# antoyang/FrozenBiLM

Hardware: AMD Instinct MI355X
Metric: video-text samples/sec (MLM fwd+bwd) DeBERTa-XL+adapters (higher is better)
Workload: dtype bf16; 1 GPU; DeBERTa-v2-XLarge(24L)+adapters ds8/8, B=32/GPU, T=10x1024, L=256 (S=266), MLM fwd+bwd+allreduce+clip+Adam, dropout 0.1 live, seeded random weights; global_batch=32, seq_len=266, parallelism=dp1, dead_layer23_encoder_pass=skipped (output unused, SURVEY fact 6); FLOPs still counted

## Files before the change

### frozenbilm_amd/attn_bwd.py

```python
from __future__ import annotations

import math

import torch

from . import lib as L

BF16, F32 = torch.bfloat16, torch.float32


_RANGE = {}


def _relidx_range(S, cfg):
    key = (S, cfg.position_buckets, cfg.max_rel, cfg.att_span)
    if key not in _RANGE:
        from .model.relpos import rel_index_vector

        rv = rel_index_vector(S, cfg.position_buckets, cfg.max_rel, cfg.att_span)
        _RANGE[key] = (int(rv[0]), int(rv[-1]) - int(rv[0]) + 1)
    return _RANGE[key]


_DRANGE = {}
POS_GRAD_MAX_DELTAS = 8


def _delta_ranges(S, cfg, dev, limit=POS_GRAD_MAX_DELTAS):
    key = (S, cfg.position_buckets, cfg.max_rel, cfg.att_span, str(dev))
    if key not in _DRANGE:
        import numpy as np

        from .model.relpos import rel_index_vector

        rv = np.asarray(rel_index_vector(S, cfg.position_buckets, cfg.max_rel, cfg.att_span), dtype=np.int64)
        rmin, rcnt = int(rv[0]), int(rv[-1]) - int(rv[0]) + 1
        first = np.searchsorted(rv, np.arange(rmin, rmin + rcnt), side="left")
        last = np.searchsorted(rv, np.arange(rmin, rmin + rcnt), side="right")
        dlo = (first - (S - 1)).astype(np.int16)
        dcnt = (last - first).astype(np.int16)
        _DRANGE[key] = (torch.from_numpy(dlo).to(dev), torch.from_numpy(dcnt).to(dev), int(dcnt.max()))
    cmax = _DRANGE[key][2]
    if limit is not None and cmax > limit:
        raise NotImplementedError(
            f"position-table gradients (fbl_attn_pos_grad) take at most {limit} relative positions per table "
            f"row; position_buckets={cfg.position_buckets}, max_relative_positions={cfg.max_rel} at sequence length {S} "
            f"puts {cmax} on one row")
    return _DRANGE[key]


def disent_attn_bwd(eng, run, sv, dctx, dqkv, dpqk, defer_pos=False):
    B, S, H, nh, span2 = run.B, run.S, eng.H, eng.nh, eng.span2
    Sp = (S + 63) // 64 * 64
    dev = eng.dev
    qkv = sv.qkv
    q, k, v = qkv[:, :H], qkv[:, H:2 * H], qkv[:, 2 * H:]
    pq, pk = sv.pqk[:, :H], sv.pqk[:, H:]
    relidx = eng.relidx(S)
    klen = getattr(run, "klen", None)
    border = getattr(run, "border", None)
    scale = 1.0 / math.sqrt(64 * 3)
    pk_ = getattr(run, "pk", None)
    row0 = pk_.row0 if pk_ is not None else None
    saved_p = getattr(sv, "psave", None) is not None

    Dv = torch.empty(B, nh, S, dtype=F32, device=dev)
    PKX = torch.empty(nh, 2 * Sp, 64, dtype=BF16, device=dev)
    if saved_p:
        QT = PQT = None
        PQX = torch.empty(nh, 2 * Sp, 64, dtype=BF16, device=dev)
    else:
        QT = torch.empty(nh, 64, B, Sp, dtype=BF16, device=dev)
        PQT = torch.empty(nh, 64, span2, dtype=BF16, device=dev)
        PQX = None
    L.attn_bwd_prep(q, pq, pk, dctx, sv.ctx, QT, PQT, Dv, B, S, Sp, nh, span2, row0=row0, relidx=relidx, PQX=PQX, PKX=PKX)
    dS = torch.empty(B, nh, Sp, Sp, dtype=BF16, device=dev)
    dST = torch.empty(B, nh, Sp, Sp, dtype=BF16, device=dev)
    lin = eng.cfg.position_buckets // 2 if eng.cfg.position_buckets > 0 else eng.cfg.att_span - 1
    if saved_p:
        L.disent_attn_bwd_dspk(sv.psave, sv.msave, q, v, dctx, PQX, sv.lse, Dv, scale, dqkv[:, H:2 * H], dqkv[:, 2 * H:], dS, dST,
                               B, S, Sp, nh, p_drop=run.p_att, seed=sv.seed_att, klen=klen, border=border, row0=row0)
        sv.psave = sv.msave = None
    else:
        lin_a = min(lin, span2 // 2) if eng.cfg.position_buckets > 0 else 0
        L.disent_attn_bwd_ds(q, k, v, dctx, pk, pq, relidx, run.mask_i32, sv.lse, Dv, scale, dqkv[:, 2 * H:], dS, dST,
                             B, S, Sp, nh, span2, p_drop=run.p_att, seed=sv.seed_att, klen=klen, border=border, lin=lin_a, row0=row0)
    L.disent_attn_bwd_dq(dS, k, PKX, dqkv[:, :H], B, S, Sp, nh, klen=klen, border=border, row0=row0)
    if not saved_p:
        L.disent_attn_bwd_shear(dST, QT, PQT, relidx, dqkv[:, H:2 * H], B, S, Sp, nh, span2, klen=klen, lin=lin, border=border,
                                row0=row0)
    rmin, rcnt = _relidx_range(S, eng.cfg)
    state = dict(dS=dS, dST=dST, q=q, k=k, rmin=rmin, rcnt=rcnt, B=B, S=S, Sp=Sp, klen=klen, row0=row0)
    if defer_pos:
        return state
    dpqk.copy_(pos_table_grads(eng, state))
    return None


def pos_table_grads(eng, st):
    H, nh, span2 = eng.H, eng.nh, eng.span2
    rmin, rcnt, B, Sp = st["rmin"], st["rcnt"], st["B"], st["Sp"]
    dpos = torch.zeros(span2, 2 * H, dtype=F32, device=eng.dev)
    dlo, dcnt, cmax = _delta_ranges(st["S"], eng.cfg, eng.dev, limit=None)
    for neg, X, Y, col0 in ((0, st["dS"], st["q"], H), (1, st["dST"], st["k"], 0)):
        d = torch.empty(1, nh, rcnt, 64, dtype=F32, device=eng.dev)
        L.attn_pos_grad(neg, [X], [Y], dlo, dcnt, cmax, d, B, st["S"], Sp, nh, rcnt, klen=st["klen"], row0=st["row0"])
        dpos[rmin:rmin + rcnt, col0:col0 + H].view(rcnt, nh, 64).copy_(d[0].permute(1, 0, 2))
    return dpos


def pos_chain_buffers(eng, run, n_exec):
    rmin, rcnt = _relidx_range(run.S, eng.cfg)
    Sp = (run.S + 63) // 64 * 64
    return dict(X1=[], X2=[], Yq=[], Yk=[], rmin=rmin, rcnt=rcnt, B=run.B, S=run.S, Sp=Sp, n=0, seeds=[], cap=n_exec, klen=None,
                row0=None)


def pos_table_grads_batched(eng, run, pc):
    H, nh, span2 = eng.H, eng.nh, eng.span2
    E, rmin, rcnt, B, Sp = pc["n"], pc["rmin"], pc["rcnt"], pc["B"], pc["Sp"]
    dev = eng.dev
    dpb = torch.empty(E, rcnt, 2 * H, dtype=BF16, device=dev)
    dlo, dcnt, cmax = _delta_ranges(pc["S"], eng.cfg, dev, limit=None)
    for neg, kx, ky, col0 in ((0, "X1", "Yq", H), (1, "X2", "Yk", 0)):
        d = torch.empty(E, nh, rcnt, 64, dtype=F32, device=dev)
        L.attn_pos_grad(neg, pc[kx][:E], pc[ky][:E], dlo, dcnt, cmax, d, B, pc["S"], Sp, nh, rcnt, klen=pc["klen"], row0=pc["row0"])
        L.heads_to_rows_bf16(d, dpb[:, :, col0:col0 + H])
    tmp = torch.empty(E, rcnt, H, dtype=F32, device=dev)
    L.gemm(dpb, eng.WposT_exec[:E], out_f32=tmp)
    dR = L.zeros(span2, H, dtype=F32, device=dev)
    L.dropout_sum_f32(tmp, pc["seeds"][:E] if run.p_hid > 0 else [0] * E, run.p_hid, dR[rmin:rmin + rcnt], key0=rmin * H)
    return dR
```

### frozenbilm_amd/csrc/attn_bwd.hip

```cpp
#include "attn_common.h"
#include "../../include/fbl.h"

namespace {
using namespace attn;

__global__ void rowdot_kernel(const bf16* dO, const bf16* O, long ld, float* out, int B, int S, int nh) {
  const long gid = (long)blockIdx.x * blockDim.x + threadIdx.x;
  const long idx = gid >> 3;
  const int c = (int)(gid & 7);
  const long total = (long)B * S * nh;
  const bool live = idx < total;
  const long row = live ? idx / nh : 0;
  const int h = live ? (int)(idx % nh) : 0;
  float s = 0.f;
  if (live) {
    const bf16x8 x = *(const bf16x8*)(dO + row * ld + h * 64 + c * 8);
    const bf16x8 y = *(const bf16x8*)(O + row * ld + h * 64 + c * 8);
#pragma unroll
    for (int e = 0; e < 8; ++e) s += bf2f(x[e]) * bf2f(y[e]);
  }
  s += __shfl_xor(s, 1, 64);
  s += __shfl_xor(s, 2, 64);
  s += __shfl_xor(s, 4, 64);
  if (live && c == 0) {
// ... 136 lines not shown
__host__ __device__ constexpr int a_total(int Sp) { return A_IDX + 2 * Sp * 2; }
static_assert(64 * LTW * 2 >= 64 * LDV * 2, "dS staging tile must fit in the T1 region");

struct ATileRegs {
  bf16x8 q[2], d[2];
  float lse, D;
};

template <bool DEVSEED, bool PACKED = false>
__global__ __launch_bounds__(256, 3) void attn_bwd_ds_kernel(BwdAArgs a) {
  extern __shared__ __attribute__((aligned(16))) char smem[];
  const int tid = threadIdx.x, lane = tid & 63;
  const int w = __builtin_amdgcn_readfirstlane(tid >> 6);
  const int c = lane & 15, g = lane >> 4;
  const int S = a.S, Sp = a.Sp;
  const WgCoord wc = wg_coord(Sp / 64, a.nh, a.B, a.border);
  const int j0 = wc.x * 64, h = wc.h, b = wc.b;
  const int j = j0 + w * 16 + c;
  const long rb = PACKED ? (long)a.row0[b] : (long)b * S;
  const int lim = PACKED ? min(a.row0[b + 1] - a.row0[b], S) : S;
  const int jc = min(j, lim - 1);
  const int tq = Sp - 1;

  int16_t* idx = (int16_t*)(smem + A_IDX);
  f16* T1 = (f16*)(smem + A_T1);
  f16* T2 = (f16*)(smem + A_T2);
  float* rlse = (float*)(smem + A_ROW);
  float* rD = rlse + 64;
  float* kms = rlse + 128;
  bf16* dst = (bf16*)(smem + A_T1);
  bf16* dstT = (bf16*)(smem + A_T2);

  const int kl = a.klen ? min(a.klen[b], S) : S;
  const int nqt = (j0 < kl) ? (kl + 63) / 64 : 0;
  const int srow = tid >> 3, sch = tid & 7;
  const int fb0 = c * 128 + ((g ^ (c & 7)) << 4), fb1 = fb0 ^ 64;
  const int sb = srow * 128 + ((sch ^ (srow & 7)) << 4);

  bf16x8 vf[2];
  {
    const long off = (rb + jc) * a.ldq + h * 64 + g * 8;
    vf[0] = *(const bf16x8*)(a.v + off);
    vf[1] = *(const bf16x8*)(a.v + off + 32);
  }
  if (nqt > 0) {
    load_idx_padded(idx, a.relidx, S, Sp, tid, 256);
#pragma unroll
    for (int t = 0; t < 2; ++t)
      *(bf16x8*)(smem + A_KS + sb + t * 4096) =
          *(const bf16x8*)(a.k + (rb + min(j0 + srow + t * 32, lim - 1)) * a.ldq + h * 64 + sch * 8);
    if (tid < 64) kms[tid] = (j0 + tid < S && a.mask[(long)b * S + min(j0 + tid, S - 1)] != 0) ? 1.f : 0.f;
    for (int t = tid; t < (2 * 64 * LTW * 2) / 16; t += 256) *(bf16x8*)(smem + A_T1 + t * 16) = (bf16x8){0, 0, 0, 0, 0, 0, 0, 0};
  }

  f32x4 dv[4];
#pragma unroll
  for (int dt = 0; dt < 4; ++dt) dv[dt] = (f32x4){0.f, 0.f, 0.f, 0.f};
  const DropKey dk = attn_drop_key(DEVSEED ? a.seed + *a.seed_dev : a.seed, b * a.nh + h, a.p_drop);
  const float k2 = a.scale * LOG2E;
  const long sbase = ((long)b * a.nh + h) * Sp * Sp;
  const int izero = a.relidx[S - 1];
  const bf16* pkh = a.pk + h * 64 + g * 8;
  const bf16* pqh = a.pq + h * 64 + g * 8;
  const int my_t0 = (0x5243 >> (w * 4)) & 15, my_t1 = (0x1670 >> (w * 4)) & 15;

  auto load_qd = [&](int it, ATileRegs& R) {
    const int i0 = it * 64;
#pragma unroll
    for (int t = 0; t < 2; ++t) {
      const int i = min(i0 + srow + t * 32, lim - 1);
      R.q[t] = *(const bf16x8*)(a.q + (rb + i) * a.ldq + h * 64 + sch * 8);
      R.d[t] = *(const bf16x8*)(a.dO + (rb + i) * a.ldo + h * 64 + sch * 8);
    }
    R.lse = INFINITY; R.D = 0.f;
    if (tid < 64) {
      const int i = i0 + tid;
      if (i < lim) {
        const long o = ((long)b * a.nh + h) * S + i;
        R.lse = a.lse[o] * LOG2E;
        R.D = a.Dv[o];
      }
    }
  };
  auto store_tile = [&](const ATileRegs& R) {
#pragma unroll
    for (int t = 0; t < 2; ++t) {
      *(bf16x8*)(smem + A_QS + sb + t * 4096) = R.q[t];
      *(bf16x8*)(smem + A_DOS + sb + t * 4096) = R.d[t];
    }
    if (tid < 64) {
      rlse[tid] = R.lse;
      rD[tid] = R.D;
    }
  };

  for (int it = 0; it < nqt; ++it) {
    const int i0 = it * 64;
    const bool band = max(abs(i0 - (j0 + 63)), abs(i0 + 63 - j0)) < a.lin;
    int r_lo, t0q[4], t0k[4];
    if (band) {
      r_lo = izero + i0 - (j0 + 63);
#pragma unroll
      for (int x = 0; x < 4; ++x) { t0q[x] = x; t0k[x] = 3 - x; }
    } else {
      if (it == 0) __syncthreads();
      r_lo = __builtin_amdgcn_readfirstlane((int)idx[i0 - (j0 + 63) + tq]);
#pragma unroll
      for (int x = 0; x < 4; ++x) {
        t0q[x] = (__builtin_amdgcn_readfirstlane((int)idx[i0 + x * 16 - (j0 + 63) + tq]) - r_lo) >> 4;
        t0k[x] = (__builtin_amdgcn_readfirstlane((int)idx[i0 - (j0 + x * 16 + 15) + tq]) - r_lo) >> 4;
      }
    }
    const int ntile = band ? 5 : 6;
    bf16x8 apk[2][2], apq[2][2];
#pragma unroll
    for (int u = 0; u < 2; ++u) {
      const long ro = (long)min(r_lo + (u ? my_t1 : my_t0) * 16 + c, a.span2 - 1) * a.ldp;
      apk[u][0] = *(const bf16x8*)(pkh + ro);
      apk[u][1] = *(const bf16x8*)(pkh + ro + 32);
      apq[u][0] = *(const bf16x8*)(pqh + ro);
      apq[u][1] = *(const bf16x8*)(pqh + ro + 32);
    }
    {
      ATileRegs R;
      load_qd(it, R);
      store_tile(R);
    }
    __syncthreads();

    f32x4 sacc[4];
    const bf16x8 kf[2] = {*(const bf16x8*)(smem + A_KS + w * 2048 + fb0), *(const bf16x8*)(smem + A_KS + w * 2048 + fb1)};
#pragma unroll
    for (int nt = 0; nt < 4; ++nt) {
      f32x4 acc = (f32x4){0.f, 0.f, 0.f, 0.f};
      acc = __builtin_amdgcn_mfma_f32_16x16x32_bf16(*(const bf16x8*)(smem + A_QS + nt * 2048 + fb0), kf[0], acc, 0, 0, 0);
      acc = __builtin_amdgcn_mfma_f32_16x16x32_bf16(*(const bf16x8*)(smem + A_QS + nt * 2048 + fb1), kf[1], acc, 0, 0, 0);
      sacc[nt] = acc;
    }
    {
      const f16 ninf = (f16)(-INFINITY);
      f16* t1s = T1 + c * LTW + g * 4;
      f16* t2s = T2 + c * LTW + g * 4;
#pragma unroll
      for (int u = 0; u < 2; ++u) {
        const int t = u ? my_t1 : my_t0;
#pragma unroll
        for (int x = 0; x < 4; ++x) {
          const int rel1 = t - t0q[x];
          if (rel1 >= 0 && rel1 < ntile) {
            f32x4 acc = (f32x4){0.f, 0.f, 0.f, 0.f};
            acc = __builtin_amdgcn_mfma_f32_16x16x32_bf16(apk[u][0], *(const bf16x8*)(smem + A_QS + x * 2048 + fb0), acc, 0, 0, 0);
            acc = __builtin_amdgcn_mfma_f32_16x16x32_bf16(apk[u][1], *(const bf16x8*)(smem + A_QS + x * 2048 + fb1), acc, 0, 0, 0);
            *(f16x4*)(t1s + x * 16 * LTW + rel1 * 16) = to_f16x4(acc);
          }
          const int rel2 = t - t0k[x];
          if (rel2 >= 0 && rel2 < ntile) {
            f32x4 acc = (f32x4){0.f, 0.f, 0.f, 0.f};
            acc = __builtin_amdgcn_mfma_f32_16x16x32_bf16(apq[u][0], *(const bf16x8*)(smem + A_KS + x * 2048 + fb0), acc, 0, 0, 0);
            acc = __builtin_amdgcn_mfma_f32_16x16x32_bf16(apq[u][1], *(const bf16x8*)(smem + A_KS + x * 2048 + fb1), acc, 0, 0, 0);
            const f16x4 tv = to_f16x4(acc);
            *(f16x4*)(t2s + x * 16 * LTW + rel2 * 16) = kms[x * 16 + c] != 0.f ? tv : (f16x4){ninf, ninf, ninf, ninf};
          }
        }
      }
    }
    __syncthreads();

    float p[16];
    if (band) {
      const f16* t1p = T1 + g * 4 * (LTW + 1) + 63 - 16 * w - c;
      const f16* t2p = T2 + (w * 16 + c) * LTW + g * 4 + 15 - c;
#pragma unroll
      for (int nt = 0; nt < 4; ++nt)
#pragma unroll
        for (int r = 0; r < 4; ++r) {
          const float s = sacc[nt][r] + (float)t1p[nt * 16 * LTW + r * (LTW + 1)] + (float)t2p[nt * 16 + r];
          p[nt * 4 + r] = __builtin_amdgcn_exp2f(fmaf(s, k2, -rlse[nt * 16 + g * 4 + r]));
        }
    } else {
      const int16_t* ib = idx + (i0 + g * 4 - j + tq);
      int sb2 = r_lo;
#pragma unroll
      for (int x = 0; x < 4; ++x) sb2 = (w == x) ? r_lo + 16 * t0k[x] : sb2;
      const f16* t1g = T1 + g * 4 * LTW;
      const f16* t2row = T2 + (w * 16 + c) * LTW;
#pragma unroll
      for (int nt = 0; nt < 4; ++nt) {
        const int sb1 = r_lo + 16 * t0q[nt];
#pragma unroll
        for (int r = 0; r < 4; ++r) {
          const int wi = ib[nt * 16 + r];
          const int w1 = clampi(wi - sb1, 0, 95), w2 = clampi(wi - sb2, 0, 95);
          const float s = sacc[nt][r] + (float)t1g[(nt * 16 + r) * LTW + w1] + (float)t2row[w2];
          p[nt * 4 + r] = __builtin_amdgcn_exp2f(fmaf(s, k2, -rlse[nt * 16 + g * 4 + r]));
        }
      }
    }
    bf16x4 dsb[4], pfh[4];
#pragma unroll
    for (int nt = 0; nt < 4; ++nt) {
      f32x4 acc = (f32x4){0.f, 0.f, 0.f, 0.f};
      acc = __builtin_amdgcn_mfma_f32_16x16x32_bf16(*(const bf16x8*)(smem + A_DOS + nt * 2048 + fb0), vf[0], acc, 0, 0, 0);
      acc = __builtin_amdgcn_mfma_f32_16x16x32_bf16(*(const bf16x8*)(smem + A_DOS + nt * 2048 + fb1), vf[1], acc, 0, 0, 0);
      float keep[4] = {1.f, 1.f, 1.f, 1.f};
      if (a.p_drop > 0.f) {
#pragma unroll
        for (int bb = 0; bb < 2; ++bb) {
          uint32_t x, y;
          attn_drop_block(dk, (i0 + nt * 16 + g * 4 + bb * 2) >> 1, j >> 1, Sp >> 1, &x, &y);
          keep[bb * 2] = attn_drop_keep(dk, x, y, 0, j & 1);
          keep[bb * 2 + 1] = attn_drop_keep(dk, x, y, 1, j & 1);
        }
      }
#pragma unroll
      for (int r = 0; r < 4; ++r) {
        const int il = nt * 16 + g * 4 + r;
        const float pv = p[nt * 4 + r];
        dsb[nt][r] = f2bf(pv * (acc[r] * keep[r] - rD[il]) * a.scale);
        pfh[nt][r] = f2bf(pv * keep[r]);
      }
    }
    __syncthreads();
#pragma unroll
    for (int kk = 0; kk < 2; ++kk) {
      bf16x8 pf;
#pragma unroll
      for (int e = 0; e < 4; ++e) {
        pf[e] = pfh[2 * kk][e];
        pf[4 + e] = pfh[2 * kk + 1][e];
      }
#pragma unroll
      for (int dt = 0; dt < 4; ++dt) {
        const int r = g * 4 + (c >> 2);
        const int ch = dt * 2 + ((c >> 1) & 1), sub = (c & 1) * 8;
        const char* db = smem + A_DOS + r * 128 + ((ch ^ (r & 7)) << 4) + sub;
        union { tr16x4 h[2]; bf16x8 v; } u;
        u.h[0] = lds_tr16((const bf16*)(db + kk * 4096));
        u.h[1] = lds_tr16((const bf16*)(db + kk * 4096 + 2048));
        dv[dt] = __builtin_amdgcn_mfma_f32_16x16x32_bf16(u.v, pf, dv[dt], 0, 0, 0);
      }
    }
#pragma unroll
    for (int nt = 0; nt < 4; ++nt) {
      *(bf16x4*)(dstT + (w * 16 + c) * LDV + nt * 16 + g * 4) = dsb[nt];
#pragma unroll
      for (int r = 0; r < 4; ++r) dst[(nt * 16 + g * 4 + r) * LDV + w * 16 + c] = dsb[nt][r];
    }
    __syncthreads();
#pragma unroll
    for (int t = 0; t < 2; ++t) {
      const int row = srow + t * 32;
      *(bf16x8*)(a.dS + sbase + (long)(i0 + row) * Sp + j0 + sch * 8) = *(const bf16x8*)(dst + row * LDV + sch * 8);
      *(bf16x8*)(a.dST + sbase + (long)(j0 + row) * Sp + i0 + sch * 8) = *(const bf16x8*)(dstT + row * LDV + sch * 8);
    }
    __syncthreads();
  }

  if (j < lim) {
    bf16* op = a.dV + (rb + j) * a.lddv + h * 64 + g * 4;
#pragma unroll
    for (int dt = 0; dt < 4; ++dt)
      *(bf16x4*)(op + dt * 16) = (bf16x4){f2bf(dv[dt][0]), f2bf(dv[dt][1]), f2bf(dv[dt][2]), f2bf(dv[dt][3])};
  }
}

struct BwdPArgs {
  const bf16* psave; const float* msave;
  const bf16* v; long ldv;
  const bf16* dO; long ldo;
  const int32_t* klen; const int32_t* border;
  const float* lse; const float* Dv;
  float scale, p_drop; uint64_t seed; const uint64_t* seed_dev;
  bf16* dV; long lddv;
  bf16* dS; bf16* dST;
  int B, S, Sp, nh;
  const int32_t* row0;
};
constexpr int LDP = 80;

__device__ __forceinline__ int tswz(int r) { return (r & 3) | ((r >> 1) & 4); }

struct BwdPKArgs {
  BwdPArgs p;
  const bf16* q; long ldq;
  const bf16* pqx;
  bf16* dK; long lddk;
};
constexpr int LDG2 = 144;
constexpr int K_DOS = 0;
constexpr int K_QS = K_DOS + 8192;
constexpr int K_PS = K_QS + 8192;
constexpr int K_STT = K_PS + 64 * LDP * 2;
constexpr int K_G2 = K_STT + 64 * LDV * 2;
constexpr int K_TAB = K_G2 + 64 * LDG2 * 2;
constexpr int K_ROW = K_TAB + 16384;
constexpr int K_TOTAL = K_ROW + 512;
static_assert(2 * K_TOTAL <= 160 * 1024, "two workgroups per CU");

struct PKTileRegs {
  bf16x8 d[2], p[2], q[2], x[2];
  float m, l, D;
};

template <bool PACKED = false>
__global__ __launch_bounds__(256, 2) void attn_bwd_dspk_kernel(BwdPKArgs ka) {
  extern __shared__ __attribute__((aligned(16))) char smem[];
  const BwdPArgs& a = ka.p;
  const int tid = threadIdx.x, lane = tid & 63;
  const int w = __builtin_amdgcn_readfirstlane(tid >> 6);
  const int c = lane & 15, g = lane >> 4;
  const int S = a.S, Sp = a.Sp;
  const WgCoord wc = wg_coord(Sp / 64, a.nh, a.B, a.border);
  const int j0 = wc.x * 64, h = wc.h, b = wc.b;
  const int j = j0 + w * 16 + c;
  const long rb = PACKED ? (long)a.row0[b] : (long)b * S;
  const int lim = PACKED ? min(a.row0[b + 1] - a.row0[b], S) : S;
  const int jc = min(j, lim - 1);
  float* rF = (float*)(smem + K_ROW);
  float* rD = rF + 64;
  bf16* dst = (bf16*)(smem + K_PS);
  bf16* dstT = (bf16*)(smem + K_STT);
  bf16* g2 = (bf16*)(smem + K_G2) + (w * 16 + c) * LDG2;

  const int kl = a.klen ? min(a.klen[b], S) : S;
  const int nqt = (j0 < kl) ? (kl + 63) / 64 : 0;
  const int srow = tid >> 3, sch = tid & 7;
  const int fb0 = c * 128 + ((g ^ (c & 7)) << 4), fb1 = fb0 ^ 64;
  const int sb = srow * 128 + ((sch ^ (srow & 7)) << 4);
  const int sp = srow * (LDP * 2) + sch * 16;
  const int sbx = srow * 128 + ((sch ^ tswz(srow)) << 4);

  bf16x8 vf[2];
  {
    const long off = (rb + jc) * a.ldv + h * 64 + g * 8;
    vf[0] = *(const bf16x8*)(a.v + off);
    vf[1] = *(const bf16x8*)(a.v + off + 32);
  }
  f32x4 dv[4], dk[4];
#pragma unroll
  for (int dt = 0; dt < 4; ++dt) {
    dv[dt] = (f32x4){0.f, 0.f, 0.f, 0.f};
    dk[dt] = (f32x4){0.f, 0.f, 0.f, 0.f};
  }
  const DropKey dkey = attn_drop_key(a.p_drop > 0.f ? fbl_seed(a.seed, a.seed_dev) : 0, b * a.nh + h, a.p_drop);
  const long sbase = ((long)b * a.nh + h) * Sp * Sp;
  const float* mrow = a.msave + (((long)b * a.nh + h) * (Sp >> 6) + wc.x) * S;
  if (nqt > 0)
    for (int t = tid; t < (64 * LDG2 * 2) / 16; t += 256) *(bf16x8*)(smem + K_G2 + t * 16) = (bf16x8){0, 0, 0, 0, 0, 0, 0, 0};
  const int W2 = 2 * Sp;
  const int ks0 = (w < 2) ? 1 : 0;
  const __amdgpu_buffer_rsrc_t xr = buf_rsrc(ka.pqx + (long)h * W2 * 64);
  const int beta0 = (Sp - j0 - 64) >> 6;
  const __amdgpu_buffer_rsrc_t dOr = buf_rsrc(a.dO + rb * a.ldo + h * 64);
  const __amdgpu_buffer_rsrc_t qr = buf_rsrc(ka.q + rb * ka.ldq + h * 64);
  const __amdgpu_buffer_rsrc_t pr = buf_rsrc(a.psave + sbase + j0);
  const __amdgpu_buffer_rsrc_t dSr = buf_rsrc(a.dS + sbase + j0);
  const __amdgpu_buffer_rsrc_t dSTr = buf_rsrc(a.dST + sbase + (long)j0 * Sp);
  const uint32_t ldo2 = (uint32_t)(a.ldo * 2), ldq2 = (uint32_t)(ka.ldq * 2);
  const uint32_t po = (uint32_t)((srow * Sp + sch * 8) * 2);
  auto load_tile = [&](int it, PKTileRegs& R) {
    const int i0 = it * 64;
#pragma unroll
    for (int t = 0; t < 2; ++t) {
      const uint32_t ir = (uint32_t)min(i0 + srow + t * 32, lim - 1);
      R.d[t] = buf_ld16(dOr, ir * ldo2 + (uint32_t)(sch * 16), 0);
      R.p[t] = buf_ld16(pr, po + (uint32_t)(t * 32 * Sp * 2), (uint32_t)(i0 * Sp * 2));
    }
#pragma unroll
    for (int t = 0; t < 2; ++t) R.x[t] = buf_ld16(xr, (uint32_t)((srow + t * 32) * 128 + sch * 16), (uint32_t)((beta0 + it + 1) * 8192));
    {
      const int i = min(i0 + lane, lim - 1);
      const long o = ((long)b * a.nh + h) * S + i;
      R.l = a.lse[o];
      R.m = mrow[i];
      R.D = a.Dv[o];
    }
  };
  auto load_q = [&](int it, PKTileRegs& R) {
#pragma unroll
    for (int t = 0; t < 2; ++t) {
      const uint32_t ir = (uint32_t)min(it * 64 + srow + t * 32, lim - 1);
      R.q[t] = (FBL_ATTN_DBGBITS & 16) ? vf[0] : buf_ld16(qr, ir * ldq2 + (uint32_t)(sch * 16), 0);
    }
  };
  auto store_tile = [&](const PKTileRegs& R, int it_i0) {
#pragma unroll
    for (int t = 0; t < 2; ++t) {
      *(bf16x8*)(smem + K_DOS + sb + t * 4096) = R.d[t];
      *(bf16x8*)(smem + K_QS + sb + t * 4096) = R.q[t];
      *(bf16x8*)(smem + K_TAB + (((it_i0 >> 6) + beta0 + 1) & 1) * 8192 + sbx + t * 4096) = R.x[t];
      *(bf16x8*)(smem + K_PS + sp + t * (32 * LDP * 2)) = R.p[t];
    }
    if (tid < 64) {
      const bool live = it_i0 + tid < lim && R.l < INFINITY;
      rF[tid] = live ? __builtin_amdgcn_exp2f(R.m - R.l * LOG2E) : 0.f;
      rD[tid] = live ? R.D : 0.f;
    }
  };

  PKTileRegs R;
  if (nqt > 0) {
    load_tile(0, R);
    load_q(0, R);
#pragma unroll
    for (int t = 0; t < 2; ++t)
      *(bf16x8*)(smem + K_TAB + (beta0 & 1) * 8192 + sbx + t * 4096) =
          buf_ld16(xr, (uint32_t)((srow + t * 32) * 128 + sch * 16), (uint32_t)(beta0 * 8192));
  }
  for (int it = 0; it < nqt; ++it) {
    const int i0 = it * 64;
    store_tile(R, i0);
    __syncthreads();
    {
      const int itn = min(it + 1, nqt - 1);
      load_tile(itn, R);
      load_q(itn, R);
    }

    bf16x4 dsb[4], pfh[4];
#pragma unroll
    for (int nt = 0; nt < 4; ++nt) {
      union { tr16x4 t; bf16x4 v; } pu;
      pu.t = lds_tr16((const bf16*)(smem + K_PS + (nt * 16 + g * 4 + (c >> 2)) * (LDP * 2) + (w * 16 + (c & 3) * 4) * 2));
      const f32x4 f4 = *(const f32x4*)(rF + nt * 16 + g * 4);
      const f32x4 d4 = *(const f32x4*)(rD + nt * 16 + g * 4);
      f32x4 acc = (f32x4){0.f, 0.f, 0.f, 0.f};
      acc = __builtin_amdgcn_mfma_f32_16x16x32_bf16(*(const bf16x8*)(smem + K_DOS + nt * 2048 + fb0), vf[0], acc, 0, 0, 0);
      acc = __builtin_amdgcn_mfma_f32_16x16x32_bf16(*(const bf16x8*)(smem + K_DOS + nt * 2048 + fb1), vf[1], acc, 0, 0, 0);
      float keep[4];
#pragma unroll
      for (int r = 0; r < 4; ++r) keep[r] = pu.t[r] < 0 ? 0.f : dkey.inv_keep;
#pragma unroll
      for (int r = 0; r < 4; ++r) {
        const float pv = f4[r] != 0.f ? fabsf(bf2f(pu.v[r])) * f4[r] : 0.f;
        dsb[nt][r] = f2bf(pv * (acc[r] * keep[r] - d4[r]) * a.scale);
        pfh[nt][r] = f2bf(pv * keep[r]);
      }
    }
#pragma unroll
    for (int kk = 0; kk < 2; ++kk) {
      bf16x8 pf, sf;
#pragma unroll
      for (int e = 0; e < 4; ++e) {
        pf[e] = pfh[2 * kk][e];
        pf[4 + e] = pfh[2 * kk + 1][e];
        sf[e] = dsb[2 * kk][e];
        sf[4 + e] = dsb[2 * kk + 1][e];
      }
#pragma unroll
      for (int dt = 0; dt < 4; ++dt) {
        const int r = g * 4 + (c >> 2);
        const int ch = dt * 2 + ((c >> 1) & 1), sub = (c & 1) * 8;
        const int o = r * 128 + ((ch ^ (r & 7)) << 4) + sub + kk * 4096;
        union { tr16x4 h[2]; bf16x8 v; } u, uq;
        u.h[0] = lds_tr16((const bf16*)(smem + K_DOS + o));
        u.h[1] = lds_tr16((const bf16*)(smem + K_DOS + o + 2048));
        dv[dt] = __builtin_amdgcn_mfma_f32_16x16x32_bf16(u.v, pf, dv[dt], 0, 0, 0);
        if (FBL_ATTN_DBGBITS & 2) continue;
        uq.h[0] = lds_tr16((const bf16*)(smem + K_QS + o));
        uq.h[1] = lds_tr16((const bf16*)(smem + K_QS + o + 2048));
        dk[dt] = __builtin_amdgcn_mfma_f32_16x16x32_bf16(uq.v, sf, dk[dt], 0, 0, 0);
      }
    }
    {
      bf16* gs = g2 + 64 - (w * 16 + c) + g * 4;
#pragma unroll
      for (int nt = 0; nt < 4; ++nt) {
        *(bf16x4*)(dstT + (w * 16 + c) * LDV + nt * 16 + g * 4) = dsb[nt];
#pragma unroll
        for (int r = 0; r < 4; ++r) {
          dst[(nt * 16 + g * 4 + r) * LDP + w * 16 + c] = dsb[nt][r];
          if (!(FBL_ATTN_DBGBITS & 4)) gs[nt * 16 + r] = dsb[nt][r];
        }
      }
    }
    if (!(FBL_ATTN_DBGBITS & 8)) {
#pragma unroll
      for (int u = 0; u < 3; ++u) {
        const int x0 = (ks0 + u) * 32 + g * 8;
        const int slot = (((i0 >> 6) + beta0 + (x0 >> 6)) & 1) * 8192;
        const int r = (x0 & 63) + (c >> 2);
        const bf16x8 gf = *(const bf16x8*)(g2 + (ks0 + u) * 32 + g * 8);
#pragma unroll
        for (int dt = 0; dt < 4; ++dt) {
          const int ch = dt * 2 + ((c >> 1) & 1), sub = (c & 1) * 8;
          union { tr16x4 h[2]; bf16x8 v; } ut;
          ut.h[0] = lds_tr16((const bf16*)(smem + K_TAB + slot + r * 128 + ((ch ^ tswz(r)) << 4) + sub));
          ut.h[1] = lds_tr16((const bf16*)(smem + K_TAB + slot + (r + 4) * 128 + ((ch ^ tswz(r + 4)) << 4) + sub));
          dk[dt] = __builtin_amdgcn_mfma_f32_16x16x32_bf16(ut.v, gf, dk[dt], 0, 0, 0);
        }
      }
    }
    __syncthreads();
#pragma unroll
    for (int t = 0; t < 2; ++t) {
      const int row = srow + t * 32;
      buf_st16(dSr, po + (uint32_t)(t * 32 * Sp * 2), (uint32_t)(i0 * Sp * 2), *(const bf16x8*)(dst + row * LDP + sch * 8));
      buf_st16(dSTr, po + (uint32_t)(t * 32 * Sp * 2), (uint32_t)(i0 * 2), *(const bf16x8*)(dstT + row * LDV + sch * 8));
    }
  }

  if (j < lim) {
    bf16* op = a.dV + (rb + j) * a.lddv + h * 64 + g * 4;
    bf16* ok = ka.dK + (rb + j) * ka.lddk + h * 64 + g * 4;
#pragma unroll
    for (int dt = 0; dt < 4; ++dt) {
      *(bf16x4*)(op + dt * 16) = (bf16x4){f2bf(dv[dt][0]), f2bf(dv[dt][1]), f2bf(dv[dt][2]), f2bf(dv[dt][3])};
      *(bf16x4*)(ok + dt * 16) = (bf16x4){f2bf(dk[dt][0]), f2bf(dk[dt][1]), f2bf(dk[dt][2]), f2bf(dk[dt][3])};
    }
  }
}

struct BwdQArgs {
  const bf16* dS;
  const bf16* k; long ldk;
  const bf16* pkx;
  const int32_t* klen; const int32_t* border;
  bf16* dQ; long lddq;
  int B, S, Sp, nh;
  const int32_t* row0;
};
constexpr int LDG1 = 104;
constexpr int Q_DS = 0;
constexpr int Q_KS = Q_DS + 8192;
constexpr int Q_G1 = Q_KS + 8192;
constexpr int Q_TAB = Q_G1 + 64 * LDG1 * 2;
constexpr int Q_TOTAL = Q_TAB + 16384;
static_assert(3 * Q_TOTAL <= 160 * 1024, "three workgroups per CU");

template <bool PACKED = false>
__global__ __launch_bounds__(256, 3) void attn_bwd_dq_kernel(BwdQArgs a) {
  extern __shared__ __attribute__((aligned(16))) char smem[];
  const int tid = threadIdx.x, lane = tid & 63;
  const int w = __builtin_amdgcn_readfirstlane(tid >> 6);
  const int c = lane & 15, g = lane >> 4;
  const int S = a.S, Sp = a.Sp;
  const WgCoord wc = wg_coord(Sp / 64, a.nh, a.B, a.border);
  const int i0 = wc.x * 64, h = wc.h, b = wc.b;
  const int i = i0 + w * 16 + c;
  const long rb = PACKED ? (long)a.row0[b] : (long)b * S;
  const int lim = PACKED ? min(a.row0[b + 1] - a.row0[b], S) : S;
  const int kl = a.klen ? min(a.klen[b], S) : S;
  const int nkt = (i0 < kl) ? (kl + 63) / 64 : 0;
  const int srow = tid >> 3, sch = tid & 7;
  const int sb = srow * 128 + ((sch ^ tswz(srow)) << 4);
  const int ks0 = (w < 2) ? 0 : 1;
  bf16* g1 = (bf16*)(smem + Q_G1) + (w * 16 + c) * LDG1;
  const int wr = w * 16 + c;
  f32x4 dq[4];
#pragma unroll
  for (int dt = 0; dt < 4; ++dt) dq[dt] = (f32x4){0.f, 0.f, 0.f, 0.f};
  if (nkt > 0) {
    for (int t = tid; t < (64 * LDG1 * 2) / 16; t += 256) *(bf16x8*)(smem + Q_G1 + t * 16) = (bf16x8){0, 0, 0, 0, 0, 0, 0, 0};
    __syncthreads();
  }

  const long sbase = ((long)b * a.nh + h) * Sp * Sp;
  const __amdgpu_buffer_rsrc_t sr = buf_rsrc(a.dS + sbase + (long)i0 * Sp);
  const __amdgpu_buffer_rsrc_t kr = buf_rsrc(a.k + rb * a.ldk + h * 64);
  const __amdgpu_buffer_rsrc_t xr = buf_rsrc(a.pkx + (long)h * 2 * Sp * 64);
  const uint32_t so = (uint32_t)((wr * Sp + g * 16) * 2);
  const uint32_t ldk2 = (uint32_t)(a.ldk * 2);
  const int beta0 = (i0 - 64 + Sp) >> 6;

  struct Regs { bf16x8 s[2], k[2], x[2]; } R;
  auto load_pair = [&](int jt) {
#pragma unroll
    for (int t = 0; t < 2; ++t) {
      R.s[t] = buf_ld16(sr, so + (uint32_t)(t * 16), (uint32_t)(jt * 128));
      const uint32_t jr = (uint32_t)min(jt * 64 + srow + t * 32, lim - 1);
      R.k[t] = buf_ld16(kr, jr * ldk2 + (uint32_t)(sch * 16), 0);
      R.x[t] = buf_ld16(xr, (uint32_t)((srow + t * 32) * 128 + sch * 16), (uint32_t)((beta0 - jt) * 8192));
    }
  };
  if (nkt > 0) {
    load_pair(0);
#pragma unroll
    for (int t = 0; t < 2; ++t)
      *(bf16x8*)(smem + Q_TAB + ((beta0 + 1) & 1) * 8192 + sb + t * 4096) =
          buf_ld16(xr, (uint32_t)((srow + t * 32) * 128 + sch * 16), (uint32_t)((beta0 + 1) * 8192));
  }
  for (int jt = 0; jt < nkt; ++jt) {
#pragma unroll
    for (int t = 0; t < 2; ++t) {
      *(bf16x8*)(smem + Q_KS + sb + t * 4096) = R.k[t];
      *(bf16x8*)(smem + Q_TAB + ((beta0 - jt) & 1) * 8192 + sb + t * 4096) = R.x[t];
      *(bf16x8*)(smem + Q_DS + wr * 128 + (((2 * g + t) ^ (wr & 7)) << 4)) = R.s[t];
    }
    {
      bf16* gs = g1 + wr + 64 - g * 16 - ks0 * 32;
#pragma unroll
      for (int t = 0; t < 2; ++t)
#pragma unroll
        for (int e = 0; e < 8; ++e) gs[-(t * 8 + e)] = R.s[t][e];
    }
    __syncthreads();
    load_pair(min(jt + 1, nkt - 1));
#pragma unroll
    for (int kk = 0; kk < 2; ++kk) {
      const int rk = kk * 32 + g * 8 + (c >> 2);
      const bf16x8 sf = *(const bf16x8*)(smem + Q_DS + wr * 128 + (((kk * 4 + g) ^ (wr & 7)) << 4));
#pragma unroll
      for (int dt = 0; dt < 4; ++dt) {
        const int ch = dt * 2 + ((c >> 1) & 1), sub = (c & 1) * 8;
        union { tr16x4 h[2]; bf16x8 v; } u;
        u.h[0] = lds_tr16((const bf16*)(smem + Q_KS + rk * 128 + ((ch ^ tswz(rk)) << 4) + sub));
        u.h[1] = lds_tr16((const bf16*)(smem + Q_KS + (rk + 4) * 128 + ((ch ^ tswz(rk + 4)) << 4) + sub));
        dq[dt] = __builtin_amdgcn_mfma_f32_16x16x32_bf16(u.v, sf, dq[dt], 0, 0, 0);
      }
    }
#pragma unroll
    for (int u3 = 0; u3 < 3; ++u3) {
      const int x0 = (ks0 + u3) * 32 + g * 8;
      const int slot = ((beta0 - jt + (x0 >> 6)) & 1) * 8192;
      const int r = (x0 & 63) + (c >> 2);
      const bf16x8 gf = *(const bf16x8*)(g1 + u3 * 32 + g * 8);
#pragma unroll
      for (int dt = 0; dt < 4; ++dt) {
        const int ch = dt * 2 + ((c >> 1) & 1), sub = (c & 1) * 8;
        union { tr16x4 h[2]; bf16x8 v; } ut;
        ut.h[0] = lds_tr16((const bf16*)(smem + Q_TAB + slot + r * 128 + ((ch ^ tswz(r)) << 4) + sub));
        ut.h[1] = lds_tr16((const bf16*)(smem + Q_TAB + slot + (r + 4) * 128 + ((ch ^ tswz(r + 4)) << 4) + sub));
        dq[dt] = __builtin_amdgcn_mfma_f32_16x16x32_bf16(ut.v, gf, dq[dt], 0, 0, 0);
      }
    }
    __syncthreads();
  }
  if (i < lim) {
    bf16* op = a.dQ + (rb + i) * a.lddq + h * 64 + g * 4;
#pragma unroll
    for (int dt = 0; dt < 4; ++dt)
      *(bf16x4*)(op + dt * 16) = (bf16x4){f2bf(dq[dt][0]), f2bf(dq[dt][1]), f2bf(dq[dt][2]), f2bf(dq[dt][3])};
  }
}

struct ShearArgs {
  const bf16* X;
  const bf16* YT; long y_sh, y_sb, y_sd;
  const bf16* PT;
  const int16_t* relidx;
  const int32_t* klen;
  const int32_t* border;
  bf16* out; long ldout;
  int B, S, Sp, nh, span2, Wg;
  int lin;
  const int32_t* row0;
};
__device__ __forceinline__ void gt_window(const int16_t* relidx, int S, int kl, int r0, int Wg, int* rbase, int* nks) {
  const int hi = 2 * S - 2;
  const int dlo = -(r0 + 31), dhi = kl - 1 - r0;
  const int rb = (int)relidx[min(max(dlo + S - 1, 0), hi)] & ~7;
  const int rt = (int)relidx[min(max(dhi + S - 1, 0), hi)];
  *rbase = rb;
  *nks = min((rt - rb + 32) / 32, Wg / 32);
}
constexpr int C_IDX = 0;
constexpr int C_G = C_IDX + 2048;

template <bool PACKED = false>
__global__ __launch_bounds__(128) void attn_bwd_shear_kernel(ShearArgs a) {
  extern __shared__ __attribute__((aligned(16))) char smem[];
  const int tid = threadIdx.x, lane = tid & 63;
  const int w = __builtin_amdgcn_readfirstlane(tid >> 6);
  const int c = lane & 15, g = lane >> 4;
  const int S = a.S, Sp = a.Sp;
  const WgCoord wc = wg_coord(Sp / 32, a.nh, a.B, a.border);
  const int r0 = wc.x * 32, h = wc.h, b = wc.b;
  const int LDG = a.Wg + 8;
  const int rl = w * 16 + c;
  const int row = r0 + rl;
  bf16* G = (bf16*)(smem + C_G);
  int16_t* idx = (int16_t*)(smem + C_IDX);
  const bf16x8 z8 = {0, 0, 0, 0, 0, 0, 0, 0};
  const int kl = a.klen ? min(a.klen[b], S) : S;
  const long rb = PACKED ? (long)a.row0[b] : (long)b * S;
  const int lim = PACKED ? min(a.row0[b + 1] - a.row0[b], S) : S;
  if (r0 >= kl) {
    if (row < lim) {
      bf16* op = a.out + (rb + row) * a.ldout + h * 64 + g * 4;
#pragma unroll
      for (int dt = 0; dt < 4; ++dt) *(bf16x4*)(op + dt * 16) = (bf16x4){0, 0, 0, 0};
    }
    return;
  }
  int rbase, nks;
  gt_window(a.relidx, S, kl, r0, a.Wg, &rbase, &nks);
  const int izero = (int)a.relidx[S - 1];
  {
    const int vpr = nks * 4;
    for (int t = tid; t < 32 * vpr; t += 128) *(bf16x8*)(G + (t / vpr) * LDG + (t % vpr) * 8) = z8;
  }
  attn::load_idx_padded(idx, a.relidx, S, Sp, tid, 128);
  const long xbase = (((long)b * a.nh + h) * Sp + row) * Sp;
  f32x4 acc[4];
#pragma unroll
  for (int dt = 0; dt < 4; ++dt) acc[dt] = (f32x4){0.f, 0.f, 0.f, 0.f};
  __syncthreads();

  const int nct = (kl + 63) / 64;
  const bf16* ytb = a.YT + h * a.y_sh + b * a.y_sb + (long)c * a.y_sd + g * 8;
  const int16_t* ib = idx + (Sp - 1 - row + g * 8);
  bf16* grow = G + rl * LDG - rbase;
  const int wmax = rbase + nks * 32 - 1;
  const int dummy = rbase + a.Wg;
  const int lin0 = izero + g * 8 - row;
  const int rw = r0 + w * 16;
  struct Frags { bf16x8 y[8], x[2]; };
  auto load_ct = [&](int ct, Frags& F) {
    const int c0 = ct * 64;
#pragma unroll
    for (int kk = 0; kk < 2; ++kk)
#pragma unroll
      for (int dt = 0; dt < 4; ++dt)
        F.y[kk * 4 + dt] = (FBL_ATTN_DBGBITS & 2048) ? z8 : *(const bf16x8*)(ytb + (long)(dt * 16) * a.y_sd + c0 + kk * 32);
    F.x[0] = *(const bf16x8*)(a.X + xbase + c0 + g * 8);
    F.x[1] = *(const bf16x8*)(a.X + xbase + c0 + 32 + g * 8);
  };
  auto step = [&](int ct, const Frags& F) {
    const int c0 = ct * 64;
    const int d_a = rw - (c0 + 63), d_b = rw + 15 - c0;
    const bool band = max(abs(d_a), abs(d_b)) < a.lin;
#pragma unroll
    for (int kk = 0; kk < 2; ++kk) {
      const bf16x8 xv = F.x[kk];
#pragma unroll
      for (int dt = 0; dt < 4; ++dt) acc[dt] = __builtin_amdgcn_mfma_f32_16x16x32_bf16(F.y[kk * 4 + dt], xv, acc[dt], 0, 0, 0);
      const int cb = c0 + kk * 32;
      if (FBL_ATTN_DBGBITS & 512) continue;
      if (band) {
        const int s0 = lin0 + cb;
#pragma unroll
        for (int e = 0; e < 8; ++e) {
          const int slot = s0 + e;
          grow[bf2f(xv[e]) != 0.f ? slot : dummy] = xv[e];
        }
      } else {
#pragma unroll
        for (int e = 0; e < 8; ++e) {
          const float x = bf2f(xv[e]);
          if (x != 0.f) {
            const int dlt = cb + g * 8 + e - row;
            const int gi = clampi((int)ib[cb + e], rbase, wmax);
            if (abs(dlt) < a.lin) {
              grow[gi] = xv[e];
            } else {
              bf16x2 pv = {(bf16)0.f, (bf16)0.f};
              pv[gi & 1] = xv[e];
              __builtin_amdgcn_ds_atomic_fadd_v2bf16((__attribute__((address_space(3))) bf16x2*)(grow + (gi & ~1)), pv);
            }
          }
        }
      }
    }
  };
  {
    Frags F0, F1;
    load_ct(0, F0);
    for (int ct = 0; ct < nct; ct += 2) {
      if (ct + 1 < nct) load_ct(ct + 1, F1);
      step(ct, F0);
      if (ct + 2 < nct) load_ct(ct + 2, F0);
      if (ct + 1 < nct) step(ct + 1, F1);
    }
  }
  const bf16* pt = a.PT + (long)h * 64 * a.span2 + rbase + g * 8;
  auto load_pt = [&](int kk, bf16x8* dstf) {
#pragma unroll
    for (int dt = 0; dt < 4; ++dt) {
      const bool ok = rbase + kk * 32 + g * 8 + 8 <= a.span2;
      dstf[dt] = ok ? *(const bf16x8*)(pt + (long)(dt * 16 + c) * a.span2 + kk * 32) : z8;
    }
  };
  auto table_step = [&](int kk, const bf16x8* af) {
    const bf16x8 bfv = *(const bf16x8*)(G + rl * LDG + kk * 32 + g * 8);
#pragma unroll
    for (int dt = 0; dt < 4; ++dt) acc[dt] = __builtin_amdgcn_mfma_f32_16x16x32_bf16(af[dt], bfv, acc[dt], 0, 0, 0);
  };
  bf16x8 pa[4], pb[4];
  const int nks_run = (FBL_ATTN_DBGBITS & 1024) ? 0 : nks;
  load_pt(0, pa);
  for (int kk = 0; kk < nks_run; kk += 2) {
    if (kk + 1 < nks) load_pt(kk + 1, pb);
    table_step(kk, pa);
    if (kk + 2 < nks) load_pt(kk + 2, pa);
    if (kk + 1 < nks) table_step(kk + 1, pb);
  }
  if (row < lim) {
    bf16* op = a.out + (rb + row) * a.ldout + h * 64 + g * 4;
#pragma unroll
    for (int dt = 0; dt < 4; ++dt)
      *(bf16x4*)(op + dt * 16) = (bf16x4){f2bf(acc[dt][0]), f2bf(acc[dt][1]), f2bf(acc[dt][2]), f2bf(acc[dt][3])};
  }
}

constexpr int PG_MAX_E = 64;
struct PosGradArgs {
  const bf16* X[PG_MAX_E];
  const bf16* Y[PG_MAX_E];
  long ldy;
  const int16_t* dlo;
  const int16_t* dcnt;
  const int32_t* klen;
  const int32_t* row0;
  float* out;
  int E, B, S, Sp, nh, rcnt;
  int cmax;
};
constexpr int PG_PAD = 48;
constexpr int PG_LDY = 80;
constexpr int PG_TPW = 4;
constexpr int PG_WAVES = 4, PG_THR = PG_WAVES * 64;
constexpr int PG_ROWS = PG_WAVES * PG_TPW * 16;
__host__ __device__ constexpr int pg_pitch(int Sp) { return Sp + 2 * PG_PAD; }
__host__ __device__ constexpr int pg_buf(int Sp) { return 32 * pg_pitch(Sp) * 2 + 32 * PG_LDY * 2; }
__host__ __device__ constexpr int pg_smem(int Sp) { return 2 * pg_buf(Sp); }

template <bool NEG, int CM, int NXR, int OCC>
__global__ __launch_bounds__(PG_THR, OCC) void pos_grad_kernel(PosGradArgs a) {
  extern __shared__ __attribute__((aligned(16))) char smem[];
  const int tid = threadIdx.x, lane = tid & 63;
  const int w = __builtin_amdgcn_readfirstlane(tid >> 6);
  const int c = lane & 15, g = lane >> 4;
  const int S = a.S, Sp = a.Sp, P = pg_pitch(Sp);
  const int nsplit = (a.rcnt + PG_ROWS - 1) / PG_ROWS;
  const int L8 = blockIdx.x >> 3, xcd = blockIdx.x & 7;
  const int prob = (L8 / nsplit) * 8 + xcd, part = L8 % nsplit;
  if (prob >= a.E * a.nh) return;
  const int e = prob / a.nh, h = prob % a.nh;
  const int bufsz = pg_buf(Sp);
  const bf16* X = a.X[e];
  const bf16* Y = a.Y[e];
  const int ntiles = (a.rcnt + 15) / 16;

  int d0[PG_TPW], dn[PG_TPW], tlo[PG_TPW], thi[PG_TPW];
  bool simple[PG_TPW];
#pragma unroll
  for (int u = 0; u < PG_TPW; ++u) {
    const int t = (w + PG_WAVES * u) * nsplit + part;
    const int r = min(t * 16 + c, a.rcnt - 1);
    const bool live = t < ntiles && t * 16 + c < a.rcnt;
    d0[u] = live ? (int)a.dlo[r] : 0;
    dn[u] = live ? (int)a.dcnt[r] : 0;
    const int rf = min(t * 16, a.rcnt - 1), rl = min(t * 16 + 15, a.rcnt - 1);
    tlo[u] = t < ntiles ? (int)a.dlo[rf] : 1 << 20;
    thi[u] = t < ntiles ? (int)a.dlo[rl] + (int)a.dcnt[rl] - 1 : -(1 << 20);
    simple[u] = t < ntiles && t * 16 + 15 < a.rcnt && (thi[u] - tlo[u]) == 15 && __builtin_amdgcn_ballot_w64(dn[u] != 1) == 0;
  }
  f32x4 acc[PG_TPW][4];
#pragma unroll
  for (int u = 0; u < PG_TPW; ++u)
#pragma unroll
    for (int dt = 0; dt < 4; ++dt) acc[u][dt] = (f32x4){0.f, 0.f, 0.f, 0.f};

  for (int id = tid; id < (OCC >= 3 ? 1 : 2) * 32 * 2 * (PG_PAD / 8); id += PG_THR) {
    const int bsel = id / (32 * 2 * (PG_PAD / 8)), r2 = id % (32 * 2 * (PG_PAD / 8));
    const int row = r2 / (2 * (PG_PAD / 8)), q = r2 % (2 * (PG_PAD / 8));
    const int col = q < PG_PAD / 8 ? q * 8 : PG_PAD + Sp + (q - PG_PAD / 8) * 8;
    *(bf16x8*)((bf16*)(smem + bsel * bufsz) + row * P + col) = (bf16x8){0, 0, 0, 0, 0, 0, 0, 0};
  }
  const bf16x8 z8 = (bf16x8){0, 0, 0, 0, 0, 0, 0, 0};
  const int srow = tid >> 3, sch = tid & 7, nq = Sp >> 6;

  int b_n = 0, k_n = 0, kl_n = 0;
  auto seek = [&]() {
    while (b_n < a.B) {
      kl_n = a.klen ? min(a.klen[b_n], S) : S;
      if (k_n < kl_n) return true;
      ++b_n; k_n = 0;
    }
    return false;
  };
  bf16x8 rx[NXR], ry;
  int it_b = 0, it_k = 0, it_kl = 0;
  auto load_item = [&]() {
    it_b = b_n; it_k = k_n; it_kl = kl_n;
    const int kl64 = (kl_n + 63) & ~63;
    const long rb = a.row0 ? (long)a.row0[b_n] : (long)b_n * S;
    const int lim = a.row0 ? min(a.row0[b_n + 1] - a.row0[b_n], S) : S;
    const bf16* Xb = X + (((long)b_n * a.nh + h) * Sp) * Sp + (long)k_n * Sp;
    const bf16* xr = Xb + (long)srow * Sp + sch * 8;
#pragma unroll
    for (int q = 0; q < NXR; ++q) rx[q] = (q < nq && sch * 8 + q * 64 < kl64) ? *(const bf16x8*)(xr + q * 64) : z8;
    {
      const int pos = k_n + srow;
      ry = (pos < lim) ? *(const bf16x8*)(Y + (rb + pos) * a.ldy + h * 64 + sch * 8) : z8;
    }
    k_n += 32;
  };
  int pb = 0;
  bool have = seek();
  if (have) load_item();
  while (have) {
    bf16* xs = (bf16*)(smem + pb * bufsz);
    bf16* ys = xs + 32 * P;
    if (OCC >= 3) __syncthreads();
    {
      bf16* xw = xs + srow * P + PG_PAD + sch * 8;
#pragma unroll
      for (int q = 0; q < NXR; ++q)
        if (q < nq) *(bf16x8*)(xw + q * 64) = rx[q];
    }
    *(bf16x8*)(ys + srow * PG_LDY + sch * 8) = ry;
    const int k0 = it_k, kl = it_kl;
    __syncthreads();
    have = seek();
    if (have) load_item();
    bf16x8 yf[4];
#pragma unroll
    for (int dt = 0; dt < 4; ++dt) {
      const bf16* yb = ys + (g * 8 + (c >> 2)) * PG_LDY + dt * 16 + (c & 3) * 4;
      union { tr16x4 hh[2]; bf16x8 v; } u2;
      u2.hh[0] = lds_tr16(yb);
      u2.hh[1] = lds_tr16(yb + 4 * PG_LDY);
      yf[dt] = u2.v;
    }
#pragma unroll
    for (int u = 0; u < PG_TPW; ++u) {
      const int cmin = NEG ? k0 + tlo[u] : k0 - thi[u];
      const int cmax = NEG ? k0 + 31 + thi[u] : k0 + 31 - tlo[u];
      if (cmax < 0 || cmin >= kl) continue;
      bf16x8 gf;
      const bf16* xrow = xs + (g * 8) * P + PG_PAD;
      const int cb = NEG ? (k0 + g * 8 + d0[u]) : (k0 + g * 8 - d0[u]);
      if (simple[u]) {
#pragma unroll
        for (int q = 0; q < 8; ++q) gf[q] = xrow[q * P + cb + q];
      } else {
        const int lo = -PG_PAD, hi = Sp + PG_PAD - 1;
        bf16 vv[8][CM];
#pragma unroll
        for (int q = 0; q < 8; ++q)
#pragma unroll
          for (int t2 = 0; t2 < CM; ++t2) vv[q][t2] = xrow[q * P + clampi(NEG ? cb + q + t2 : cb + q - t2, lo, hi)];
#pragma unroll
        for (int q = 0; q < 8; ++q) {
          float sum = 0.f;
#pragma unroll
          for (int t2 = 0; t2 < CM; ++t2) sum += t2 < dn[u] ? bf2f(vv[q][t2]) : 0.f;
          gf[q] = f2bf(sum);
        }
      }
#pragma unroll
      for (int dt = 0; dt < 4; ++dt) acc[u][dt] = __builtin_amdgcn_mfma_f32_16x16x32_bf16(yf[dt], gf, acc[u][dt], 0, 0, 0);
    }
    if (OCC < 3) pb ^= 1;
  }
  float* ob = a.out + ((long)e * a.nh + h) * a.rcnt * 64;
#pragma unroll
  for (int u = 0; u < PG_TPW; ++u) {
    const int r = ((w + PG_WAVES * u) * nsplit + part) * 16 + c;
    if (r < a.rcnt) {
#pragma unroll
      for (int dt = 0; dt < 4; ++dt) *(f32x4*)(ob + (long)r * 64 + dt * 16 + g * 4) = acc[u][dt];
    }
  }
}

constexpr int PGW_PAD = 6;
__host__ __device__ constexpr int pgw_pitch(int Sp) { return Sp + PGW_PAD; }
__host__ __device__ constexpr int pgw_smem(int Sp) { return 32 * pgw_pitch(Sp) * 4 + 32 * PG_LDY * 2; }

template <bool NEG>
__global__ __launch_bounds__(PG_THR, 2) void pos_grad_wide_kernel(PosGradArgs a) {
  extern __shared__ __attribute__((aligned(16))) char smem[];
  const int tid = threadIdx.x, lane = tid & 63;
  const int w = __builtin_amdgcn_readfirstlane(tid >> 6);
  const int c = lane & 15, g = lane >> 4;
  const int S = a.S, Sp = a.Sp, PP = pgw_pitch(Sp);
  const int nsplit = (a.rcnt + PG_ROWS - 1) / PG_ROWS;
  const int L8 = blockIdx.x >> 3, xcd = blockIdx.x & 7;
  const int prob = (L8 / nsplit) * 8 + xcd, part = L8 % nsplit;
  if (prob >= a.E * a.nh) return;
  const int e = prob / a.nh, h = prob % a.nh;
  float* cs = (float*)smem;
  bf16* ys = (bf16*)(smem + 32 * PP * 4);
  const bf16* X = a.X[e];
  const bf16* Y = a.Y[e];
  const int ntiles = (a.rcnt + 15) / 16;

  int d0[PG_TPW], dn[PG_TPW], tlo[PG_TPW], thi[PG_TPW];
#pragma unroll
  for (int u = 0; u < PG_TPW; ++u) {
    const int t = (w + PG_WAVES * u) * nsplit + part;
    const int r = min(t * 16 + c, a.rcnt - 1);
    const bool live = t < ntiles && t * 16 + c < a.rcnt;
    d0[u] = live ? (int)a.dlo[r] : 0;
    dn[u] = live ? (int)a.dcnt[r] : 0;
    const int rf = min(t * 16, a.rcnt - 1), rl = min(t * 16 + 15, a.rcnt - 1);
    tlo[u] = t < ntiles ? (int)a.dlo[rf] : 1 << 20;
    thi[u] = t < ntiles ? (int)a.dlo[rl] + (int)a.dcnt[rl] - 1 : -(1 << 20);
  }
  f32x4 acc[PG_TPW][4];
#pragma unroll
  for (int u = 0; u < PG_TPW; ++u)
#pragma unroll
    for (int dt = 0; dt < 4; ++dt) acc[u][dt] = (f32x4){0.f, 0.f, 0.f, 0.f};

  if (tid < 32) cs[tid * PP + 1] = 0.f;
  const bf16x8 z8 = (bf16x8){0, 0, 0, 0, 0, 0, 0, 0};
  const int srow = tid >> 3, sch = tid & 7, nq = Sp >> 6;

  int b_n = 0, k_n = 0, kl_n = 0;
  auto seek = [&]() {
    while (b_n < a.B) {
      kl_n = a.klen ? min(a.klen[b_n], S) : S;
      if (k_n < kl_n) return true;
      ++b_n; k_n = 0;
    }
    return false;
  };
  bf16x8 rx[8], ry;
  int it_k = 0, it_kl = 0;
  auto load_item = [&]() {
    it_k = k_n; it_kl = kl_n;
    const int kl64 = (kl_n + 63) & ~63;
    const long rb = a.row0 ? (long)a.row0[b_n] : (long)b_n * S;
    const int lim = a.row0 ? min(a.row0[b_n + 1] - a.row0[b_n], S) : S;
    const bf16* xr = X + (((long)b_n * a.nh + h) * Sp) * Sp + (long)(k_n + srow) * Sp + sch * 8;
#pragma unroll
    for (int q = 0; q < 8; ++q) rx[q] = (q < nq && sch * 8 + q * 64 < kl64) ? *(const bf16x8*)(xr + q * 64) : z8;
    const int pos = k_n + srow;
    ry = (pos < lim) ? *(const bf16x8*)(Y + (rb + pos) * a.ldy + h * 64 + sch * 8) : z8;
    k_n += 32;
  };
  bool have = seek();
  if (have) load_item();
  while (have) {
    __syncthreads();
    {
      float* cw = cs + srow * PP + 2 + sch * 8;
      float carry = 0.f;
#pragma unroll
      for (int q = 0; q < 8; ++q) {
        if (q < nq) {
          float run[8];
          run[0] = bf2f(rx[q][0]);
#pragma unroll
          for (int i = 1; i < 8; ++i) run[i] = run[i - 1] + bf2f(rx[q][i]);
          float incl = run[7];
#pragma unroll
          for (int s = 1; s < 8; s <<= 1) {
            const float o = __shfl_up(incl, s, 8);
            if (sch >= s) incl += o;
          }
          const float excl = __shfl_up(incl, 1, 8);
          const float base = carry + (sch ? excl : 0.f);
#pragma unroll
          for (int i = 0; i < 8; i += 2) *(float2*)(cw + q * 64 + i) = make_float2(base + run[i], base + run[i + 1]);
          carry += __shfl(incl, 7, 8);
        }
      }
    }
    *(bf16x8*)(ys + srow * PG_LDY + sch * 8) = ry;
    const int k0 = it_k, kl = it_kl;
    __syncthreads();
    have = seek();
    if (have) load_item();
    bf16x8 yf[4];
#pragma unroll
    for (int dt = 0; dt < 4; ++dt) {
      const bf16* yb = ys + (g * 8 + (c >> 2)) * PG_LDY + dt * 16 + (c & 3) * 4;
      union { tr16x4 hh[2]; bf16x8 v; } u2;
      u2.hh[0] = lds_tr16(yb);
      u2.hh[1] = lds_tr16(yb + 4 * PG_LDY);
      yf[dt] = u2.v;
    }
    const float* crow = cs + (g * 8) * PP + 1;
#pragma unroll
    for (int u = 0; u < PG_TPW; ++u) {
      const int cmin = NEG ? k0 + tlo[u] : k0 - thi[u];
      const int cmax = NEG ? k0 + 31 + thi[u] : k0 + 31 - tlo[u];
      if (cmax < 0 || cmin >= kl) continue;
      const int kb = k0 + g * 8;
      float hi[8], lo[8];
#pragma unroll
      for (int q = 0; q < 8; ++q) {
        const int jl = NEG ? kb + q + d0[u] : kb + q - d0[u] - dn[u] + 1;
        hi[q] = crow[q * PP + clampi(jl + dn[u], 0, Sp)];
        lo[q] = crow[q * PP + clampi(jl, 0, Sp)];
      }
      bf16x8 gf;
#pragma unroll
      for (int q = 0; q < 8; ++q) gf[q] = f2bf(hi[q] - lo[q]);
#pragma unroll
      for (int dt = 0; dt < 4; ++dt) acc[u][dt] = __builtin_amdgcn_mfma_f32_16x16x32_bf16(yf[dt], gf, acc[u][dt], 0, 0, 0);
    }
  }
  float* ob = a.out + ((long)e * a.nh + h) * a.rcnt * 64;
#pragma unroll
  for (int u = 0; u < PG_TPW; ++u) {
    const int r = ((w + PG_WAVES * u) * nsplit + part) * 16 + c;
    if (r < a.rcnt) {
#pragma unroll
      for (int dt = 0; dt < 4; ++dt) *(f32x4*)(ob + (long)r * 64 + dt * 16 + g * 4) = acc[u][dt];
    }
  }
}

}

extern "C" int fbl_attn_rowdot(const void* dO, const void* O, int64_t ld, float* out, int B, int S, int nh,
                               void* stream) {
  if (ld % 8) return FBL_ERR_ALIGN;
  const long total = (long)B * S * nh;
  if (total <= 0) return 0;
  hipLaunchKernelGGL(rowdot_kernel, dim3((unsigned)((total * 8 + 255) / 256)), dim3(256), 0, (hipStream_t)stream,
                     (const bf16*)dO, (const bf16*)O, (long)ld, out, B, S, nh);
  FBL_CHECK_LAUNCH();
  return 0;
}

extern "C" int fbl_disent_attn_bwd_ds(const void* q, const void* k, const void* v, int64_t ldq, const void* dO,
                                      int64_t ldo,
                                      const void* pk, const void* pq, int64_t ldp, const int16_t* relidx,
                                      const int32_t* mask, const int32_t* klen, const int32_t* border, const float* lse, const float* Dv, float scale, float p_drop,
                                      uint64_t seed, const uint64_t* seed_dev, void* dV, int64_t lddv, void* dS, void* dST, int B, int S, int Sp,
                                      int nh, int span2, int lin_span, const int32_t* row0, void* stream) {
  if (S < 1 || S > 512 || Sp < S || Sp % 64) return FBL_ERR_SHAPE;
  if ((ldq % 8) || (ldo % 8) || (ldp % 8) || (lddv % 4)) return FBL_ERR_ALIGN;
  if (lin_span < 0 || 2 * lin_span > span2) return FBL_ERR_ARG;
  if (row0 && !klen) return FBL_ERR_ARG;
  if (B <= 0 || nh <= 0) return 0;
  BwdAArgs a{(const bf16*)q, (const bf16*)k, (const bf16*)v, ldq, (const bf16*)dO, ldo, (const bf16*)pk, (const bf16*)pq, ldp, relidx, mask, klen, border, lse, Dv, scale, p_drop, seed, (bf16*)dV, lddv,
             (bf16*)dS, (bf16*)dST, B, S, Sp, nh, span2, lin_span, seed_dev, row0};
  attn_debug_init();
  const int smem_bytes = a_total(Sp);
  static int attr_bytes = 0;
  if (smem_bytes > attr_bytes) {
    hipError_t e = hipFuncSetAttribute((const void*)attn_bwd_ds_kernel<false>, hipFuncAttributeMaxDynamicSharedMemorySize, smem_bytes);
    if (e == hipSuccess) e = hipFuncSetAttribute((const void*)attn_bwd_ds_kernel<true>, hipFuncAttributeMaxDynamicSharedMemorySize, smem_bytes);
    if (e == hipSuccess) e = hipFuncSetAttribute((const void*)attn_bwd_ds_kernel<false, true>, hipFuncAttributeMaxDynamicSharedMemorySize, smem_bytes);
    if (e == hipSuccess) e = hipFuncSetAttribute((const void*)attn_bwd_ds_kernel<true, true>, hipFuncAttributeMaxDynamicSharedMemorySize, smem_bytes);
    if (e != hipSuccess) return (int)e;
    attr_bytes = smem_bytes;
  }
  const dim3 grid((unsigned)(Sp / 64) * nh * B);
  const bool devseed = seed_dev && p_drop > 0.f;
  if (row0 && devseed)
    hipLaunchKernelGGL((attn_bwd_ds_kernel<true, true>), grid, dim3(256), smem_bytes, (hipStream_t)stream, a);
  else if (row0)
    hipLaunchKernelGGL((attn_bwd_ds_kernel<false, true>), grid, dim3(256), smem_bytes, (hipStream_t)stream, a);
  else if (devseed)
    hipLaunchKernelGGL(attn_bwd_ds_kernel<true>, grid, dim3(256), smem_bytes, (hipStream_t)stream, a);
  else
    hipLaunchKernelGGL(attn_bwd_ds_kernel<false>, grid, dim3(256), smem_bytes, (hipStream_t)stream, a);
  FBL_CHECK_LAUNCH();
  return 0;
}

extern "C" int fbl_disent_attn_bwd_dspk(const void* psave, const float* msave, const void* q, int64_t ldq, const void* v, int64_t ldv,
                                        const void* dO, int64_t ldo, const void* pqx, const int32_t* klen, const int32_t* border,
                                        const float* lse, const float* Dv, float scale, float p_drop, uint64_t seed,
                                        const uint64_t* seed_dev, void* dK, int64_t lddk, void* dV, int64_t lddv, void* dS, void* dST,
                                        int B, int S, int Sp, int nh, const int32_t* row0, void* stream) {
  if (S < 1 || S > 512 || Sp < S || Sp % 64) return FBL_ERR_SHAPE;
  if ((ldv % 8) || (ldo % 8) || (ldq % 8) || (lddv % 4) || (lddk % 4)) return FBL_ERR_ALIGN;
  if (!psave || !msave || !q || !v || !dO || !pqx || !lse || !Dv || !dK || !dV || !dS || !dST) return FBL_ERR_ARG;
  if (row0 && !klen) return FBL_ERR_ARG;
  if (B <= 0 || nh <= 0) return 0;
  BwdPKArgs a{{(const bf16*)psave, msave, (const bf16*)v, ldv, (const bf16*)dO, ldo, klen, border, lse, Dv, scale, p_drop, seed,
               seed_dev, (bf16*)dV, lddv, (bf16*)dS, (bf16*)dST, B, S, Sp, nh, row0},
              (const bf16*)q, ldq, (const bf16*)pqx, (bf16*)dK, lddk};
  attn_debug_init();
  static bool attr_set = false;
  if (!attr_set) {
    hipError_t e = hipFuncSetAttribute((const void*)attn_bwd_dspk_kernel<false>, hipFuncAttributeMaxDynamicSharedMemorySize, K_TOTAL);
    if (e == hipSuccess) e = hipFuncSetAttribute((const void*)attn_bwd_dspk_kernel<true>, hipFuncAttributeMaxDynamicSharedMemorySize, K_TOTAL);
    if (e != hipSuccess) return (int)e;
    attr_set = true;
  }
  const dim3 grid((unsigned)(Sp / 64) * nh * B);
  if (row0)
    hipLaunchKernelGGL(attn_bwd_dspk_kernel<true>, grid, dim3(256), K_TOTAL, (hipStream_t)stream, a);
  else
    hipLaunchKernelGGL(attn_bwd_dspk_kernel<false>, grid, dim3(256), K_TOTAL, (hipStream_t)stream, a);
  FBL_CHECK_LAUNCH();
  return 0;
}

extern "C" int fbl_disent_attn_bwd_dq(const void* dS, const void* k, int64_t ldk, const void* pkx, const int32_t* klen,
                                      const int32_t* border, void* dQ, int64_t lddq, int B, int S, int Sp, int nh,
                                      const int32_t* row0, void* stream) {
  if (S < 1 || S > 512 || Sp < S || Sp % 64) return FBL_ERR_SHAPE;
  if ((ldk % 8) || (lddq % 4)) return FBL_ERR_ALIGN;
  if (!dS || !k || !pkx || !dQ) return FBL_ERR_ARG;
  if (row0 && !klen) return FBL_ERR_ARG;
  if (B <= 0 || nh <= 0) return 0;
  BwdQArgs a{(const bf16*)dS, (const bf16*)k, ldk, (const bf16*)pkx, klen, border, (bf16*)dQ, lddq, B, S, Sp, nh, row0};
  static bool attr_set = false;
  if (!attr_set) {
    hipError_t e = hipFuncSetAttribute((const void*)attn_bwd_dq_kernel<false>, hipFuncAttributeMaxDynamicSharedMemorySize, Q_TOTAL);
    if (e == hipSuccess) e = hipFuncSetAttribute((const void*)attn_bwd_dq_kernel<true>, hipFuncAttributeMaxDynamicSharedMemorySize, Q_TOTAL);
    if (e != hipSuccess) return (int)e;
    attr_set = true;
  }
  const dim3 grid((unsigned)(Sp / 64) * nh * B);
  if (row0)
    hipLaunchKernelGGL(attn_bwd_dq_kernel<true>, grid, dim3(256), Q_TOTAL, (hipStream_t)stream, a);
  else
    hipLaunchKernelGGL(attn_bwd_dq_kernel<false>, grid, dim3(256), Q_TOTAL, (hipStream_t)stream, a);
  FBL_CHECK_LAUNCH();
  return 0;
}

extern "C" int fbl_disent_attn_bwd_shear(const void* dST, const void* QT, int64_t y_sh, int64_t y_sb, int64_t y_sd,
                                         const void* PQT, const int16_t* relidx, const int32_t* klen, const int32_t* border,
                                         void* dK, int64_t lddk, int lin_span, int B, int S, int Sp, int nh, int span2,
                                         const int32_t* row0, void* stream) {
  if (S < 1 || S > 512 || Sp < S || Sp % 64 || span2 > 512 || span2 % 32) return FBL_ERR_SHAPE;
  if ((lddk % 4) || (y_sd % 8) || (y_sb % 8) || (y_sh % 8)) return FBL_ERR_ALIGN;
  if (B <= 0 || nh <= 0) return 0;
  int Wg = S + 31 + 7;
  if (Wg > span2) Wg = span2;
  Wg = (Wg + 31) / 32 * 32;
  if (row0 && !klen) return FBL_ERR_ARG;
  ShearArgs a{(const bf16*)dST, (const bf16*)QT, y_sh, y_sb, y_sd, (const bf16*)PQT, relidx, klen, border, (bf16*)dK, lddk,
              B, S, Sp, nh, span2, Wg, lin_span, row0};
  attn_debug_init();
  const int smem_bytes = C_G + 32 * (Wg + 8) * 2;
  static int attr_bytes = 0;
  if (smem_bytes > attr_bytes) {
    hipError_t e = hipFuncSetAttribute((const void*)attn_bwd_shear_kernel<false>, hipFuncAttributeMaxDynamicSharedMemorySize, smem_bytes);
    if (e == hipSuccess) e = hipFuncSetAttribute((const void*)attn_bwd_shear_kernel<true>, hipFuncAttributeMaxDynamicSharedMemorySize, smem_bytes);
    if (e != hipSuccess) return (int)e;
    attr_bytes = smem_bytes;
  }
  dim3 grid((unsigned)(Sp / 32) * nh * B);
  if (row0)
    hipLaunchKernelGGL(attn_bwd_shear_kernel<true>, grid, dim3(128), smem_bytes, (hipStream_t)stream, a);
  else
    hipLaunchKernelGGL(attn_bwd_shear_kernel<false>, grid, dim3(128), smem_bytes, (hipStream_t)stream, a);
  FBL_CHECK_LAUNCH();
  return 0;
}

extern "C" int fbl_attn_pos_grad(int neg, const void* const* X, const void* const* Y, int64_t ldy, const int16_t* dlo,
                                 const int16_t* dcnt, int dcnt_max, const int32_t* klen, const int32_t* row0, float* out, int E,
                                 int B, int S, int Sp, int nh, int rcnt, void* stream) {
  if (S < 1 || S > 512 || Sp < S || Sp % 64 || rcnt < 1 || rcnt > 1024) return FBL_ERR_SHAPE;
  if (ldy % 8) return FBL_ERR_ALIGN;
  if (!X || !Y || !dlo || !dcnt || !out || dcnt_max < 1) return FBL_ERR_ARG;
  if (row0 && !klen) return FBL_ERR_ARG;
  if (E <= 0 || B <= 0 || nh <= 0) return 0;
  for (int e = 0; e < E; ++e)
    if (!X[e] || !Y[e]) return FBL_ERR_ARG;
  static const int occ_sw = FBL_ENV_INT("FBL_POSGRAD_OCC", 3);
  const bool occ3 = Sp <= 320 && dcnt_max <= 3 && occ_sw >= 3;
  const int smem_bytes = occ3 ? pg_buf(Sp) : pg_smem(Sp);
  static int attr_bytes = 0;
  if (pg_smem(Sp) > attr_bytes) {
    const void* fns[6] = {(const void*)pos_grad_kernel<false, 3, 5, 3>, (const void*)pos_grad_kernel<true, 3, 5, 3>,
                          (const void*)pos_grad_kernel<false, 3, 8, 2>, (const void*)pos_grad_kernel<true, 3, 8, 2>,
                          (const void*)pos_grad_kernel<false, 8, 8, 2>, (const void*)pos_grad_kernel<true, 8, 8, 2>};
    for (int i = 0; i < 6; ++i) {
      hipError_t e1 = hipFuncSetAttribute(fns[i], hipFuncAttributeMaxDynamicSharedMemorySize, pg_smem(Sp));
      if (e1 != hipSuccess) return (int)e1;
    }
    attr_bytes = pg_smem(Sp);
  }
  const bool wide = dcnt_max > 8;
  static int attr_wide = 0;
  if (wide && pgw_smem(Sp) > attr_wide) {
    for (const void* fn : {(const void*)pos_grad_wide_kernel<false>, (const void*)pos_grad_wide_kernel<true>}) {
      hipError_t e1 = hipFuncSetAttribute(fn, hipFuncAttributeMaxDynamicSharedMemorySize, pgw_smem(Sp));
      if (e1 != hipSuccess) return (int)e1;
    }
    attr_wide = pgw_smem(Sp);
  }
  const int nsplit = (rcnt + PG_ROWS - 1) / PG_ROWS;
  for (int e0 = 0; e0 < E; e0 += PG_MAX_E) {
    PosGradArgs a{};
    const int ne = E - e0 < PG_MAX_E ? E - e0 : PG_MAX_E;
    for (int e = 0; e < ne; ++e) {
      a.X[e] = (const bf16*)X[e0 + e];
      a.Y[e] = (const bf16*)Y[e0 + e];
    }
    a.ldy = ldy; a.dlo = dlo; a.dcnt = dcnt; a.klen = klen; a.row0 = row0;
    a.out = out + (long)e0 * nh * rcnt * 64;
    a.E = ne; a.B = B; a.S = S; a.Sp = Sp; a.nh = nh; a.rcnt = rcnt; a.cmax = dcnt_max;
    const dim3 grid((unsigned)(((ne * nh + 7) / 8) * 8 * nsplit));
#define FBL_PG_LAUNCH(NEG_, CM_, NXR_, OCC_) \
  hipLaunchKernelGGL((pos_grad_kernel<NEG_, CM_, NXR_, OCC_>), grid, dim3(PG_THR), smem_bytes, (hipStream_t)stream, a)
    if (wide) {
      if (neg) hipLaunchKernelGGL(pos_grad_wide_kernel<true>, grid, dim3(PG_THR), pgw_smem(Sp), (hipStream_t)stream, a);
      else hipLaunchKernelGGL(pos_grad_wide_kernel<false>, grid, dim3(PG_THR), pgw_smem(Sp), (hipStream_t)stream, a);
    } else if (occ3) {
      if (neg) FBL_PG_LAUNCH(true, 3, 5, 3);
      else FBL_PG_LAUNCH(false, 3, 5, 3);
    } else if (dcnt_max <= 3) {
      if (neg) FBL_PG_LAUNCH(true, 3, 8, 2);
      else FBL_PG_LAUNCH(false, 3, 8, 2);
    } else {
      if (neg) FBL_PG_LAUNCH(true, 8, 8, 2);
      else FBL_PG_LAUNCH(false, 8, 8, 2);
    }
#undef FBL_PG_LAUNCH
    FBL_CHECK_LAUNCH();
  }
  return 0;
}

extern "C" int fbl_attn_bwd_prep(const void* q, int64_t ldq, const void* pq, const void* pk, int64_t ldp, const void* dO,
                                 const void* O, int64_t ldo, void* QT, void* PQT, float* Dv, const int16_t* relidx, void* PQX,
                                 void* PKX, int B, int S, int Sp, int nh, int span2, const int32_t* row0, void* stream) {
  if (S < 1 || Sp < S || Sp % 64 || span2 <= 0 || span2 % 64) return FBL_ERR_SHAPE;
  if ((ldq % 8) || (ldp % 8) || (ldo % 8)) return FBL_ERR_ALIGN;
  if ((PQX || PKX) && !relidx) return FBL_ERR_ARG;
  if (!Dv) return FBL_ERR_ARG;
  if (B <= 0 || nh <= 0) return 0;
  const int n_tr = (Sp / 64) * nh * B, n_tab = (span2 / 64) * nh, n_x = (2 * Sp / 64) * nh;
  PrepArgs a{(const bf16*)q, ldq, (const bf16*)pq, (const bf16*)pk, ldp, (const bf16*)dO, (const bf16*)O, ldo, (bf16*)QT,
             (bf16*)PQT, Dv, B, S, Sp, nh, span2, QT ? n_tr : 0, PQT ? n_tab : 0, row0, relidx, (bf16*)PQX, (bf16*)PKX,
             PQX ? n_x : 0, PKX ? n_x : 0};
  const long n_dot = ((long)B * S * nh * 8 + 255) / 256;
  const long grid = (long)a.n_qt + a.n_pqt + a.n_pqx + a.n_pkx + n_dot;
  hipLaunchKernelGGL(attn_bwd_prep_kernel, dim3((unsigned)grid), dim3(256), 0, (hipStream_t)stream, a);
  FBL_CHECK_LAUNCH();
  return 0;
}
```

### frozenbilm_amd/engine.py

```python
from __future__ import annotations

import math
from dataclasses import dataclass, field
from typing import Dict, List, Optional

import numpy as np
import torch

from . import lib as L
from .model.relpos import rel_index_vector

BF16, F32 = torch.bfloat16, torch.float32


def _ru(x: int, m: int) -> int:
    return (x + m - 1) // m * m


@dataclass
class NormRef:
    t: torch.Tensor
    stats: torch.Tensor
    gamma: torch.Tensor
    beta: torch.Tensor
    rowmask: Optional[torch.Tensor] = None

    def as_args(self):
        return (self.t, self.stats, self.gamma, self.beta, self.rowmask)


@dataclass
class Stream:
    bf16: torch.Tensor
    norm: Optional[NormRef] = None
    plain: Optional[torch.Tensor] = None
    full: Optional[torch.Tensor] = None


@dataclass
class Packing:
    row0: torch.Tensor
    sel: torch.Tensor
    inv: torch.Tensor
    pos: torch.Tensor
    n: int


class Engine:
    def __init__(self, model):
        self.m = model
        cfg = model.config
        self.cfg = cfg
        self.H, self.I, self.V = cfg.hidden_size, cfg.intermediate_size, cfg.vocab_size
        self.nh = cfg.num_attention_heads
        self.nL = cfg.num_hidden_layers
        self.span2 = 2 * cfg.att_span
        self.lin_span = min(cfg.position_buckets // 2, cfg.att_span) if cfg.position_buckets > 0 else 0
        self.F = model.features_dim
        self.Fp = _ru(self.F, 64) if self.F else 0
        self.A1 = self.H // model.ds_factor_attn if model.ds_factor_attn else 0
        self.A2 = self.H // model.ds_factor_ff if model.ds_factor_ff else 0
        self.Vp = _ru(self.V, 64)
        dev = model.device
        if dev.type != "cuda":
            raise RuntimeError("frozenbilm_amd runs on MI355X only: move the model to a cuda (HIP) device; "
                               "there is no CPU fallback")
        L.load()
        self.dev = dev
        self.opts = dict(getattr(model, "engine_options", None) or {})
        unknown = set(self.opts) - {"eager_logits", "side_stream", "fold_dx", "dw_on_side", "fuse_tail", "merge", "dw_group", "attn_save_p"}
        if unknown:
            raise ValueError(f"unknown engine_options: {sorted(unknown)}")
        self._build_flat()
        self._pack_frozen()
        self._relidx: Dict[int, torch.Tensor] = {}
        self._pos_cache: Dict[int, torch.Tensor] = {}
        self._no_pos_cache = False
        self.reducer = None
        self._pad_bufs = {}
        self._dyz_pool: Dict[tuple, list] = {}
        self._dyz_shape = None
        self.params_version = 0
        self._ops_version = None
        self.skip_dead_layer = True
        self._ln_ws = L.ln_bwd_ws(self.H, dev)
        self._cs_ws = L.colsum_ws(max(self.H, self.I), dev)
        self.sk_ws = torch.empty(48 << 20, dtype=F32, device=dev)
        self.side = torch.cuda.Stream(device=dev)
        if L._AUX.get(dev.index if dev.index is not None else torch.cuda.current_device()) is None:
            L.set_aux_stream(torch.cuda.Stream(device=dev), dev)
        o = self.opts
        self.eager_logits = bool(o.get("eager_logits", False))
        self.side_ws = torch.empty(8 << 20, dtype=F32, device=dev)
        self.side_cs_ws = L.colsum_ws(max(self.H, self.I), dev)
        self.use_side_stream = bool(o.get("side_stream", True))
        self.fold_dx = bool(o.get("fold_dx", True))
        self.dw_on_side = bool(o.get("dw_on_side", False))
        self.attn_save_p = bool(o.get("attn_save_p", True))
        self.fuse_tail = bool(o.get("fuse_tail", True))
        L.exclude_from_aux(self.side)
        self.dw_group = max(1, min(L.ADW_MAX_ADAPTERS, int(o.get("dw_group", 16))))

    def _build_flat(self):
        from .model.deberta import flat_order

        m = self.m
        named = dict(m.named_parameters())
        train_names = [n for n, p in named.items() if p.requires_grad]
        order = flat_order(self.cfg, train_names)
        offs, total = {}, 0
        for n in order:
            offs[n] = total
            total += _ru(named[n].numel(), 8)
        self.flat = torch.zeros(total, dtype=F32, device=self.dev)
        from .parallel import SCALAR_SLOT

        self.flat_grad_full = torch.zeros(SCALAR_SLOT + total, dtype=F32, device=self.dev)
        self.flat_grad = self.flat_grad_full[SCALAR_SLOT:]
        self.flat_bf16 = torch.zeros(total, dtype=BF16, device=self.dev)
        self.offsets, self.order = offs, order
        self._adT_offs = {}
        self.G: Dict[str, torch.Tensor] = {}
        self.Pb: Dict[str, torch.Tensor] = {}
        for n in order:
            p = named[n]
            o, k = offs[n], p.numel()
            view = self.flat[o:o + k].view(p.shape)
            view.copy_(p.data)
            p.data = view
            self.G[n] = self.flat_grad[o:o + k].view(p.shape)
            self.Pb[n] = self.flat_bf16[o:o + k].view(p.shape)
        self.P = {n: p.data for n, p in named.items()}
        self.named = named
        self.bucket_ends: Dict[str, int] = {}
        for n in order:
            key = self._bucket_key(n)
            self.bucket_ends[key] = offs[n] + _ru(named[n].numel(), 8)

    def _bucket_key(self, name: str) -> str:
        if name.startswith("lm_predictions."):
            return "head"
        if name.startswith("deberta.encoder.layer."):
            return "layer" + name.split(".")[3]
        if name.startswith("deberta.encoder.conv."):
            return "layer0" if False else "conv"
        if name.startswith("deberta.encoder.LayerNorm"):
            return "relln"
        return "emb"

    def attach_grads(self):
        fresh = all(self.named[n].grad is None for n in self.order)
        if fresh:
            L.zero_(self.flat_grad)
        for n in self.order:
            p = self.named[n]
            if p.grad is None:
                if not fresh:
                    self.G[n].zero_()
                p.grad = self.G[n]
            elif p.grad.data_ptr() != self.G[n].data_ptr():
                self.G[n].copy_(p.grad)
                p.grad = self.G[n]

    def _pack_frozen(self):
        P, H, I = self.P, self.H, self.I
        nL, dev = self.nL, self.dev
        bf = lambda t: t.to(BF16).contiguous()
        self.merge1 = bool(self.A1) and self.A1 % 64 == 0 and H % 64 == 0 and bool(self.opts.get("merge", True))
        self.merge2 = bool(self.A2) and self.A2 % 64 == 0 and H % 64 == 0 and bool(self.opts.get("merge", True))
        self.WoT_rev = torch.empty(nL, H, H, dtype=BF16, device=dev)
        self.WdT_rev = torch.empty(nL, I, H, dtype=BF16, device=dev)
        if self.merge1:
            self.Kf1 = _ru(H + self.A1, 128)
            self.WoF_rev = torch.zeros(nL, H, self.Kf1, dtype=BF16, device=dev)
            self.WoM_rev = torch.zeros(nL, H + self.A1, H, dtype=BF16, device=dev)
            self.boM_rev = torch.zeros(nL, H + self.A1, dtype=F32, device=dev)
            self.bo16_rev = torch.zeros(nL, 1, H, dtype=BF16, device=dev)
        if self.merge2:
            self.WdM_rev = torch.zeros(nL, H + self.A2, I, dtype=BF16, device=dev)
            self.bdM_rev = torch.zeros(nL, H + self.A2, dtype=F32, device=dev)
            self.bd16_rev = torch.zeros(nL, 1, H, dtype=BF16, device=dev)
        self.Lw = []
        for i in range(self.nL):
            p = f"deberta.encoder.layer.{i}"
            s = p + ".attention.self."
            j = nL - 1 - i
            Wqkv = torch.cat([P[s + "query_proj.weight"], P[s + "key_proj.weight"], P[s + "value_proj.weight"]], 0)
            self.WoT_rev[j].copy_(P[p + ".attention.output.dense.weight"].t())
            self.WdT_rev[j].copy_(P[p + ".output.dense.weight"].t())
            d = dict(
                Wqkv=bf(Wqkv), WqkvT=bf(Wqkv.t()),
                bqkv=torch.cat([P[s + "query_proj.bias"], P[s + "key_proj.bias"], P[s + "value_proj.bias"]]).float().contiguous(),
                Wo=bf(P[p + ".attention.output.dense.weight"]), WoT=self.WoT_rev[j],
                bo=P[p + ".attention.output.dense.bias"].float().contiguous(),
                Wi=bf(P[p + ".intermediate.dense.weight"]), WiT=bf(P[p + ".intermediate.dense.weight"].t()),
                bi=P[p + ".intermediate.dense.bias"].float().contiguous(),
                Wd=bf(P[p + ".output.dense.weight"]), WdT=self.WdT_rev[j],
                bd=P[p + ".output.dense.bias"].float().contiguous(),
            )
            if self.merge1:
                self.WoM_rev[j, :H].copy_(d["Wo"])
                self.boM_rev[j, :H].copy_(d["bo"])
                self.bo16_rev[j, 0].copy_(d["bo"])
                d["WoM"], d["boM"] = self.WoM_rev[j], self.boM_rev[j]
                self.WoF_rev[j, :, :H].copy_(self.WoT_rev[j])
                d["WoF"] = self.WoF_rev[j]
            if self.merge2:
                self.WdM_rev[j, :H].copy_(d["Wd"])
                self.bdM_rev[j, :H].copy_(d["bd"])
                self.bd16_rev[j, 0].copy_(d["bd"])
                d["WdM"], d["bdM"] = self.WdM_rev[j], self.bdM_rev[j]
            self.Lw.append(d)
        order = [nL - 1, nL - 1] + list(range(nL - 2, -1, -1))
        self.WposT_exec = torch.empty(len(order), H, 2 * H, dtype=BF16, device=dev)
        for e, li in enumerate(order):
            self.WposT_exec[e].copy_(self.Lw[li]["WqkvT"][:, : 2 * H])
        if self.cfg.conv_kernel_size:
            w = P["deberta.encoder.conv.conv.weight"]
            W2 = w.permute(0, 2, 1).reshape(H, 3 * H)
            self.Wc, self.WcT = bf(W2), bf(W2.t())
            self.bc = P["deberta.encoder.conv.conv.bias"].float().contiguous()
        hd = "lm_predictions.lm_head."
        self.Wh, self.WhT = bf(P[hd + "dense.weight"]), bf(P[hd + "dense.weight"].t())
        self.bh = P[hd + "dense.bias"].float().contiguous()
        E = P["deberta.embeddings.word_embeddings.weight"]
        self.E32 = E.float().contiguous()
        self.Eb = bf(E)
        self.ETb = torch.zeros(H, self.Vp, dtype=BF16, device=self.dev)
        self.ETb[:, : self.V] = E.t().to(BF16)
        self.head_bias = P[hd + "bias"].float().contiguous()
        self.rel_emb = P["deberta.encoder.rel_embeddings.weight"].float().contiguous()
        self.pos_emb = P["deberta.embeddings.position_embeddings.weight"].float().contiguous()
        if self.m.n_ans:
            T = P["answer_embeddings.weight"]
            self.n_ans = T.shape[0]
            self.Ansb = bf(T)
            self.ans_bias = P["answer_bias"].float().contiguous()

    def relidx(self, S: int) -> torch.Tensor:
        if S not in self._relidx:
            v = rel_index_vector(S, self.cfg.position_buckets, self.cfg.max_rel, self.cfg.att_span)
            self._relidx[S] = torch.from_numpy(np.ascontiguousarray(v)).to(self.dev)
        return self._relidx[S]

    def _refresh_if_stale(self, need_grad: bool):
        frozen = getattr(self.m, "_weights_frozen", 0) > 0
        ver = (self.params_version, tuple(self.named[n]._version for n in self.order)) if (frozen and not need_grad) else None
        if ver is None or ver != self._ops_version:
            self.refresh_trainable_operands()
            self._ops_version = ver

    def seed_word_value(self) -> int:
        return (self.m.dropout_seed_base() * 0x9E3779B1) & 0x7FFFFFFFFFFFFFFF

    def prepare_inference(self):
        self._refresh_if_stale(False)
        ev = getattr(self, "_compose_ev", None)
        if ev is not None:
            torch.cuda.current_stream().wait_event(ev[1])
            self._compose_ev = None

    def invalidate_operands(self):
        self._ops_version = None
        self.params_version += 1

    def refresh_trainable_operands(self):
        self._pos_cache.clear()
        L.cast_bf16(self.flat, self.flat_bf16)
        H = self.H
        self.ad = []
        for i in range(self.nL):
            p = f"deberta.encoder.layer.{i}"
            ent = {}
            for key, blk, A in (("a1", ".attention.output.adapter", self.A1), ("a2", ".output.adapter", self.A2)):
                if not A:
                    continue
                Ap = _ru(A, 64)
                down = self.Pb[p + blk + ".down.weight"]
                up = self.Pb[p + blk + ".up.weight"]
                if Ap != A:
                    upp = self._pad_bufs.get((i, key))
                    if upp is None:
                        upp = self._pad_bufs[(i, key)] = torch.zeros(H, Ap, dtype=BF16, device=self.dev)
                    upp[:, :A] = up
                    up = upp
                ent[key] = dict(down=down, up=up, A=A, Ap=Ap, name=p + blk,
                                bd=self.P[p + blk + ".down.bias"], bu=self.P[p + blk + ".up.bias"])
            self.ad.append(ent)
        if self.merge1 or self.merge2:
            if self.use_side_stream:
                self.side.wait_stream(torch.cuda.current_stream())
                with torch.cuda.stream(self.side):
                    self._compose_ev = self._compose_adapter_down(events=True)
            else:
                self._compose_adapter_down()
                self._compose_ev = None
        if self.F:
            wv = self.Pb["deberta.embeddings.linear_video.weight"]
            if self.Fp != self.F:
                w2 = self._pad_bufs.get("Wv")
                if w2 is None:
                    w2 = self._pad_bufs["Wv"] = torch.zeros(H, self.Fp, dtype=BF16, device=self.dev)
                w2[:, : self.F] = wv
                wv = w2
            self.Wv = wv

    def _compose_adapter_down(self, events=False, grad=True):
        H, nL = self.H, self.nL
        sites = []
        for on, blk, A, WT, WM, bM, b16, WF in ((self.merge1, ".attention.output.adapter", self.A1, self.WoT_rev,
                                                 getattr(self, "WoM_rev", None), getattr(self, "boM_rev", None),
                                                 getattr(self, "bo16_rev", None), getattr(self, "WoF_rev", None)),
                                                (self.merge2, ".output.adapter", self.A2, self.WdT_rev,
                                                 getattr(self, "WdM_rev", None), getattr(self, "bdM_rev", None),
                                                 getattr(self, "bd16_rev", None), None)):
            if not on:
                continue
            ow = [self.offsets[f"deberta.encoder.layer.{i}{blk}.down.weight"] for i in range(nL)]
            ob = [self.offsets[f"deberta.encoder.layer.{i}{blk}.down.bias"] for i in range(nL)]
            if nL >= 3 and len({ow[i - 1] - ow[i] for i in range(2, nL)}) == 1 and \
                    len({ob[i - 1] - ob[i] for i in range(2, nL)}) == 1 and ow[nL - 2] - ow[nL - 1] == ob[nL - 2] - ob[nL - 1] > 0:
                groups = [(nL - 1, 1, ow[0], ob[0], A * H), (0, nL - 1, ow[nL - 1], ob[nL - 1], ow[nL - 2] - ow[nL - 1])]
            else:
                groups = [(nL - 1 - i, 1, ow[i], ob[i], A * H) for i in range(nL)]
            sites.append((A, WT, WM, bM, b16, groups, WF))

        def run_group(A, WT, WM, bM, b16, grp, WF=None):
            j0, nb, o_w, o_b, st = grp
            wd3 = torch.as_strided(self.flat_bf16, (nb, A, H), (st, H, 1), o_w)
            L.gemm(wd3, WT[j0:j0 + nb], out_bf16=WM[j0:j0 + nb, H:H + A, :])
            if WF is not None and grad:
                L.gemm(WT[j0:j0 + nb], wd3, out_bf16=WF[j0:j0 + nb, :, H:H + A])
            bd3 = torch.as_strided(self.flat, (nb, A, 1), (st, 1, 1), o_b)
            bo3 = torch.as_strided(bM, (nb, A, 1), (bM.stride(0), 1, 1), bM[j0, H:].storage_offset())
            L.gemm(wd3, b16[j0:j0 + nb], aux=bd3, aux_kind=L.AUX_ADD_F32, out_f32=bo3)

        for A, WT, WM, bM, b16, groups, WF in sites:
            run_group(A, WT, WM, bM, b16, groups[0], WF)
        ev0 = ev1 = None
        if events:
            ev0 = torch.cuda.Event()
            ev0.record()
        for A, WT, WM, bM, b16, groups, WF in sites:
            for grp in groups[1:]:
                run_group(A, WT, WM, bM, b16, grp, WF)
        if events:
            ev1 = torch.cuda.Event()
            ev1.record()
            return ev0, ev1
        return None

    def _adapter_bwd_operands(self, ent):
        if "upT" not in ent:
            H = self.H
            groups = {}
            for e in self.ad:
                for key in ("a1", "a2"):
                    if key in e:
                        groups.setdefault((e[key]["A"], e[key]["Ap"]), []).append(e[key])
            for (A, Ap), ents in groups.items():
                upT_all = torch.empty(len(ents), A, H, dtype=BF16, device=self.dev)
                for i, e in enumerate(ents):
                    e["upT"] = upT_all[i]
                cache = self._adT_offs.get((A, Ap))
                if cache is None:
                    i64 = lambda v: torch.tensor(v, dtype=torch.int64, device=self.dev)
                    cache = dict(up_src=i64([self.offsets[e["name"] + ".up.weight"] for e in ents]),
                                 dn_src=i64([self.offsets[e["name"] + ".down.weight"] for e in ents]),
                                 dst=i64([i * A * H for i in range(len(ents))]))
                    self._adT_offs[(A, Ap)] = cache
                L.transpose_batched_bf16(self.flat_bf16, cache["up_src"], upT_all, cache["dst"], H, A)
                if Ap == A:
                    dnT_all = torch.empty(len(ents), H, A, dtype=BF16, device=self.dev)
                    L.transpose_batched_bf16(self.flat_bf16, cache["dn_src"], dnT_all, cache["dst"], A, H)
                    for i, e in enumerate(ents):
                        e["downT"] = dnT_all[i]
                else:
                    for e in ents:
                        downT = torch.zeros(H, Ap, dtype=BF16, device=self.dev)
                        downT[:, :A].copy_(self.Pb[e["name"] + ".down.weight"].t())
                        e["downT"] = downT
        return ent["upT"], ent["downT"]

    def run(self, input_ids, attention_mask, video, video_mask, labels, mlm, want_hidden, logit_rows=None, want_attn=False):
        m = self.m
        train = m.training
        need_grad = torch.is_grad_enabled() and any(self.named[n].requires_grad for n in self.order)
        if input_ids.device != self.dev:
            raise RuntimeError(f"inputs must be on {self.dev}")
        if attention_mask is None:
            attention_mask = torch.ones_like(input_ids)
        B, Lt = input_ids.shape
        use_video = bool(self.F) and video is not None
        T = video.shape[1] if use_video else 0
        S = T + Lt
        if S > self.cfg.max_position_embeddings:
            raise RuntimeError(
                f"sequence of {S} positions (video {T} + text {Lt}) exceeds max_position_embeddings="
                f"{self.cfg.max_position_embeddings} (the reference fails the same way, model/deberta.py:1020-1021,1392)")
        if use_video:
            if video_mask is None:
# ... 293 lines not shown
            if i == nL - 1:
                keep, run.save = run.save, False
                x = self._layer_fwd(run, i, x, None, Rb)
                run.save = keep
            else:
                x = self._layer_fwd(run, i, x, None, Rb)
            if i == 0 and cfg.conv_kernel_size:
                x = self._conv_fwd(run, emb, x)
            hs.append(x)
        kv = hs[nL - 1]
        q32 = torch.empty(N, H, dtype=F32, device=dev)
        qfull = torch.empty(N + self.span2, H, dtype=BF16, device=dev)
        if pk is None:
            self._materialize(kv, add=self.pos_emb, S=S, out_f32=q32, out_bf16=qfull[:N])
        else:
            n_ = kv.norm
            if n_ is not None:
                L.ln_materialize(n_.t, n_.stats, n_.gamma, n_.beta, rowmask=n_.rowmask, out_f32=q32)
            else:
                q32.copy_(kv.plain)
            q32.add_(self.pos_emb.index_select(0, pk.pos))
            qfull[:N].copy_(q32)
        q = Stream(bf16=qfull[:N], plain=q32, full=qfull)
        for _ in range(2):
            q = self._layer_fwd(run, nL - 1, kv, q, Rb)
        if want_hidden:
            if pk is None:
                run.hidden_out = tuple(self._materialize(s).view(B, S, H) for s in hs)
            else:
                run.hidden_out = tuple(torch.zeros(B * S, H, dtype=F32, device=dev).index_copy_(0, pk.sel, self._materialize(s))
                                       .view(B, S, H) for s in hs)
        hin = q.bf16
        rows_only = getattr(run, "logit_rows", None)
        loss_rows = (rows_only is None and run.labels is not None and not run.save and not self.eager_logits
                     and 0 < run.rows.numel() < N)
        n_all = B * S
        if loss_rows:
            run.head_in_all = q.bf16
            rows_only = run.rows.to(torch.int32)
        if rows_only is not None:
            N = rows_only.numel()
            hin = torch.empty(N, H, dtype=BF16, device=dev)
            if N:
                L.gather_rows_bf16(q.bf16, rows_only, hin)
        hp, hl = self._head_stage(run, hin, N)
        run.head_pre, run.head_norm, run.head_ln_bf16 = hp, hl.norm, hl.bf16
        if use_ans:
            Vout, table, bias = self.n_ans, self.Ansb, self.ans_bias
        else:
            Vout, table, bias = self.V, self.Eb, self.head_bias
        ldv = _ru(Vout, 64)
        run.Vout = Vout
        run.head_table, run.head_bias, run.ldv = table, bias, ldv
        if run.labels is not None:
            rows = run.rows
            run.rows_i32 = rows.to(torch.int32)
            R = rows.numel()
            run.loss_acc = L.zeros(2, dtype=F32, device=dev)
            if R > 0:
                if loss_rows:
                    hrows = hl.bf16
                else:
                    hrows = torch.empty(R, H, dtype=BF16, device=dev)
                    L.gather_rows_bf16(hl.bf16, run.rows_i32, hrows)
                lc = torch.empty(R, ldv, dtype=F32, device=dev)
                L.gemm(hrows, table, bias=bias, out_f32=lc, N=Vout)
                lab_rows = getattr(run, "label_rows", None)
                run.labels_c = run.labels[rows if lab_rows is None else lab_rows].contiguous()
                run.row_lse = torch.empty(R, dtype=F32, device=dev)
                L.ce_fwd(lc, run.labels_c, Vout, run.row_lse, run.loss_acc)
                run.logits_c = lc
            loss_t = run.loss_acc[0] / run.loss_acc[1]
            run.logits = torch.empty(n_all, ldv, dtype=F32, device=dev)
            run.logits_pending = True
            if self.eager_logits:
                self.fill_logits(run)
            return run.logits, loss_t
        logits = torch.empty(N, ldv, dtype=F32, device=dev)
        L.gemm(hl.bf16, table, bias=bias, out_f32=logits, N=Vout)
        run.logits = logits
        return logits, None

    def fill_logits(self, run):
        if getattr(run, "logits_pending", False):
            run.logits_pending = False
            hin_all = getattr(run, "head_in_all", None)
            if hin_all is not None:
                _, hl = self._head_stage(run, hin_all, hin_all.shape[0])
                run.head_ln_bf16, run.head_in_all = hl.bf16, None
            pk = getattr(run, "pk", None)
            if pk is None:
                L.gemm(run.head_ln_bf16, run.head_table, bias=run.head_bias, out_f32=run.logits, N=run.Vout)
            else:
                run.logits.zero_()
                for r0 in range(0, pk.n, 1024):
                    r1 = min(pk.n, r0 + 1024)
                    slab = torch.empty(r1 - r0, run.logits.shape[1], dtype=F32, device=self.dev)
                    L.gemm(run.head_ln_bf16[r0:r1], run.head_table, bias=run.head_bias, out_f32=slab, N=run.Vout)
                    run.logits.index_copy_(0, pk.sel[r0:r1], slab)

    def _head_stage(self, run, hin, N):
        hp = torch.empty(N, self.H, dtype=F32, device=self.dev)
        L.gemm(hin, self.Wh, bias=self.bh, out_f32=hp)
        hg = torch.empty(N, self.H, dtype=F32, device=self.dev)
        L.dropout_gelu_fwd(hp, 0.0, 0, hg)
        hl, _ = self._ln(run, "lm_predictions.lm_head.LayerNorm", y=hg, resid=None, N=N)
        return hp, hl

    def _materialize(self, s: Stream, add=None, S=1, out_f32=None, out_bf16=None):
        N, H = s.bf16.shape
        if s.plain is not None and add is None and out_bf16 is None:
            return s.plain
        if out_f32 is None:
            out_f32 = torch.empty(N, H, dtype=F32, device=self.dev)
        if s.norm is not None:
            n = s.norm
            L.ln_materialize(n.t, n.stats, n.gamma, n.beta, rowmask=n.rowmask, add_bcast=add, S=S, out_f32=out_f32,
                             out_bf16=out_bf16)
        else:
            v = s.plain if add is None else (s.plain.view(-1, S, H) + add[:S]).view(N, H)
            out_f32.copy_(v)
            if out_bf16 is not None:
                out_bf16.copy_(v)
        return out_f32

    def _conv_fwd(self, run, emb: Stream, l0: Stream) -> Stream:
        B, S, H, dev = run.B, run.S, self.H, self.dev
        N = run.N
        pk = getattr(run, "pk", None)
        if pk is None:
            col = torch.empty(N, 3 * H, dtype=BF16, device=dev)
            L.im2col3(emb.bf16, col, B, S, H)
        else:
            grid = torch.zeros(B * S, H, dtype=BF16, device=dev).index_copy_(0, pk.sel, emb.bf16)
            colg = torch.empty(B * S, 3 * H, dtype=BF16, device=dev)
            L.im2col3(grid, colg, B, S, H)
            col = colg.index_select(0, pk.sel)
        c = torch.empty(N, H, dtype=F32, device=dev)
        L.gemm(col, self.Wc, bias=self.bc, rowscale=run.mask_f, out_f32=c)
        y = torch.empty(N, H, dtype=F32, device=dev)
        run.seed_conv = run.next_seed() if run.p_hid > 0 else 0
        L.dropout_gelu_fwd(c, run.p_hid, run.seed_conv, y)
        out, _ = self._ln(run, "deberta.encoder.conv.LayerNorm", y=y, resid=l0, N=N, rowmask=run.rowmask, tail=self.span2)
        run.conv_c, run.conv_norm = c, out.norm
        return out

    def _ln_bwd(self, name, dout, norm: NormRef, p_drop, seed, want_dy_bf16=True, dysum=None, tail=0, dy_out=None):
        N, H = dout.shape
        dt_full = torch.empty(N + tail, H, dtype=F32, device=self.dev)
        dt = dt_full[:N]
        if tail:
            dt_full[N:].zero_()
        dyb = dy_out if dy_out is not None else (torch.empty(N, H, dtype=BF16, device=self.dev) if want_dy_bf16 else None)
        L.ln_bwd(dout, norm.t, norm.stats, norm.gamma, rowmask=norm.rowmask, p_drop=p_drop, seed=seed, out_dt=dt,
                 out_dy_bf16=dyb, dgamma=self.G.get(name + ".weight"), dbeta=self.G.get(name + ".bias"), dysum=dysum,
                 ws=self._ln_ws)
        if tail:
            return dt, dyb, dt_full
        return dt, dyb

    def _adapter_bwd(self, run, ent, dyb, z, xin_b, seed, dz_out=None, pooled=None):
        N, H = dyb.shape
        A, Ap = ent["A"], ent["Ap"]
        dev = self.dev
        upT, downT = self._adapter_bwd_operands(ent)
        if dz_out is not None:
            dz = dz_out
        else:
            dz = torch.zeros(N, Ap, dtype=BF16, device=dev) if Ap != A else torch.empty(N, Ap, dtype=BF16, device=dev)
        inv_keep = 1.0 / (1.0 - run.p_ad) if run.p_ad > 0 else 1.0
        L.gemm(dyb, upT, alpha=inv_keep, aux=z, aux_kind=L.AUX_MUL_POS_BF16, out_bf16=dz, N=A)
        dx = None
        if dz_out is None:
            dx = torch.empty(N, H, dtype=BF16, device=dev)
            L.gemm(dz, downT, aux=dyb, aux_kind=L.AUX_ADD_BF16, out_bf16=dx)
        sk = max(2, min(16, N // 512))
        nm = ent["name"]

        if Ap <= 256 and H % 8 == 0 and not self.dw_on_side:
            run.dw_pending.append((A, nm, (dyb, z, dz, xin_b), run.dw_count, pooled))
            run.dw_count += 1
            return dx

        def dw_work(ws, cs_ws):
            L.gemm_tn_acc(dyb, z, self.G[nm + ".up.weight"], ws, N=A, splitk=sk)
            L.gemm_tn_acc(dz, xin_b, self.G[nm + ".down.weight"], ws, M=A, splitk=sk)
            L.colsum(dz, self.G[nm + ".down.bias"], cs_ws, cols=A)

        if self.use_side_stream:
            main = torch.cuda.current_stream()
            self.side.wait_stream(main)
            with torch.cuda.stream(self.side):
                dw_work(self.side_ws, self.side_cs_ws)
            if not torch.cuda.is_current_stream_capturing():
                for t in (dyb, z, dz, xin_b):
                    t.record_stream(self.side)
            else:
                run.__dict__.setdefault("_pos_keep", []).extend((dyb, z, dz, xin_b))
            run.side_used = True
            if self.reducer is not None:
                run.dw_event = torch.cuda.Event()
                run.dw_event.record(self.side)
        else:
            dw_work(self.sk_ws, self._cs_ws)
        return dx

    def _dw_flush(self, run, red=None, force=False):
        pend = run.dw_pending
        while pend and (force or len({rec[1] for rec in pend}) >= self.dw_group):
            take, names, rest = {}, set(), []
            for rec in pend:
                A, nm, seg = rec[:3]
                if nm in names or len(names) >= min(self.dw_group, L.ADW_MAX_ADAPTERS):
                    rest.append(rec)
                else:
                    names.add(nm)
                    take.setdefault(A, []).append((nm, seg))
            for A, recs in take.items():
                L.adapter_bwd_dw([([seg], self.G[nm + ".up.weight"], self.G[nm + ".down.weight"], self.G[nm + ".down.bias"])
                                  for nm, seg in recs], A=A)
            kept = {id(r) for r in rest}
            for rec in pend:
                if id(rec) not in kept and rec[4] is not None and tuple(rec[4].shape) == self._dyz_shape:
                    self._dyz_pool.setdefault(self._dyz_shape, []).append(rec[4])
            pend[:] = rest
        if red is not None:
            parked = {self._bucket_key(rec[1] + ".up.weight") for rec in pend}
            still = []
            for key in run.dw_ready_keys:
                if key in parked:
                    still.append(key)
                else:
                    red.ready(key)
            run.dw_ready_keys[:] = still

    def _layer_bwd(self, run, sv: "LayerSave", dout: torch.Tensor):
        li = sv.li
        W, ad = self.Lw[li], self.ad[li]
        H, I, dev = self.H, self.I, self.dev
        N = dout.shape[0]
        p = f"deberta.encoder.layer.{li}"
        dt2, dy2 = self._ln_bwd(p + ".output.LayerNorm", dout, sv.ln2, run.p_hid, sv.seed_ln2,
                                dysum=self.G[ad["a2"]["name"] + ".up.bias"] if "a2" in ad else None)
        df = dy2
        if "a2" in ad:
            df = self._adapter_bwd(run, ad["a2"], dy2, sv.z2, sv.fb, sv.seed_ad2)
        dh = torch.empty(N, I, dtype=BF16, device=dev)
        L.gemm(df, W["WdT"], aux=sv.hpre, aux_kind=L.AUX_MUL_BF16, out_bf16=dh)
        da = torch.empty(N, H, dtype=F32, device=dev)
        L.gemm(dh, W["WiT"], aux=dt2, aux_kind=L.AUX_ADD_F32, out_f32=da)
        del dh
        dctx = torch.empty(N, H, dtype=BF16, device=dev)
        fold = "a1" in ad and self.fold_dx and "WoF" in W and ad["a1"]["Ap"] == ad["a1"]["A"]
        if fold:
            A1 = ad["a1"]["A"]
            pooled = None
            can_pool = (not torch.cuda.is_current_stream_capturing() and ad["a1"]["Ap"] <= 256 and H % 8 == 0 and not self.dw_on_side)
            if can_pool and self._dyz_shape != (N, self.Kf1):
                self._dyz_pool.clear()
                self._dyz_shape = (N, self.Kf1)
            free = self._dyz_pool.get((N, self.Kf1)) if can_pool else None
            if free:
                dyz = pooled = free.pop()
            elif can_pool:
                dyz = pooled = torch.zeros(N, self.Kf1, dtype=BF16, device=dev)
            else:
                dyz = torch.empty(N, self.Kf1, dtype=BF16, device=dev)
                if self.Kf1 > H + A1:
                    dyz[:, H + A1:].zero_()
            dt1, dy1 = self._ln_bwd(p + ".attention.output.LayerNorm", da, sv.ln1, run.p_hid, sv.seed_ln1,
                                    dysum=self.G[ad["a1"]["name"] + ".up.bias"], dy_out=dyz[:, :H])
            self._adapter_bwd(run, ad["a1"], dy1, sv.z1, sv.ob, sv.seed_ad1, dz_out=dyz[:, H:H + A1], pooled=pooled)
            L.gemm(dyz, W["WoF"], out_bf16=dctx)
        else:
            dt1, dy1 = self._ln_bwd(p + ".attention.output.LayerNorm", da, sv.ln1, run.p_hid, sv.seed_ln1,
                                    dysum=self.G[ad["a1"]["name"] + ".up.bias"] if "a1" in ad else None)
            do = dy1
            if "a1" in ad:
                do = self._adapter_bwd(run, ad["a1"], dy1, sv.z1, sv.ob, sv.seed_ad1)
            L.gemm(do, W["WoT"], out_bf16=dctx)
        dqkv = self._attn_bwd(run, sv, dctx)
        if not sv.emd:
            dx = torch.empty(N, H, dtype=F32, device=dev)
            L.gemm(dqkv, W["WqkvT"], aux=dt1, aux_kind=L.AUX_ADD_F32, out_f32=dx)
            return dx, None
        dq = torch.empty(N, H, dtype=F32, device=dev)
        L.gemm(dqkv[:, :H], W["WqkvT"][:, :H], aux=dt1, aux_kind=L.AUX_ADD_F32, out_f32=dq)
        return dq, dqkv[:, H:]

    def _attn_bwd(self, run, sv, dctx):
        B, S, H, nh = run.B, run.S, self.H, self.nh
        N = run.N
        dqkv = torch.empty(N, 3 * H, dtype=BF16, device=self.dev)
        from .attn_bwd import disent_attn_bwd

        if self.reducer is not None:
            self.reducer.window()

        pc = getattr(run, "pos_chain", None)
        st = disent_attn_bwd(self, run, sv, dctx, dqkv, None, defer_pos=True)
        if pc is not None:
            pc["seeds"].append(sv.seed_pos)
            pc["n"] += 1
            pc["X1"].append(st["dS"]); pc["X2"].append(st["dST"]); pc["Yq"].append(st["q"]); pc["Yk"].append(st["k"])
            pc["klen"], pc["row0"] = st["klen"], st["row0"]
        return dqkv

    def _head_bwd(self, run, rows, dlog, dq, all_rows=False):
        H, dev = self.H, self.dev
        R, Vp = dlog.shape
        Vout = run.Vout
        if Vout == self.V:
            tableT = self.ETb
        else:
            tableT = torch.zeros(H, Vp, dtype=BF16, device=dev)
            tableT[:, :Vout] = self.Ansb.t()
        dhl = L.zeros(R, H, dtype=F32, device=dev)
        if R >= 2048:
            L.gemm(dlog, tableT, out_f32=dhl)
        else:
            L.gemm(dlog, tableT, out_f32=dhl, splitk=max(2, min(16, Vp // 8192)), ws=self.sk_ws)
        rl = rows.long()
        hn = run.head_norm
        sub = NormRef(hn.t[rl].contiguous(), hn.stats[rl].contiguous(), hn.gamma, hn.beta)
        dt, _ = self._ln_bwd("lm_predictions.lm_head.LayerNorm", dhl, sub, 0.0, 0, want_dy_bf16=False)
        dpre = torch.empty(R, H, dtype=BF16, device=dev)
        L.dropout_gelu_bwd(dt, run.head_pre[rl].contiguous(), 0.0, 0, out_bf16=dpre)
        dqr = torch.empty(R, H, dtype=F32, device=dev)
        L.gemm(dpre, self.WhT, out_f32=dqr)
        if all_rows:
            dq.add_(dqr)
        else:
            L.scatter_rows_f32(dqr, rows, dq)

    def backward(self, run, gloss: Optional[torch.Tensor], glogits: Optional[torch.Tensor] = None, attach: bool = True):
        if not run.save:
            raise RuntimeError("forward was run without gradient bookkeeping")
        with L.seed_word(getattr(run, "seed_word", None)):
            return self._backward(run, gloss, glogits, attach)

    def _backward(self, run, gloss, glogits, attach):
        cfg, H, dev = self.cfg, self.H, self.dev
        B, S, T = run.B, run.S, run.T
        N = run.N
        pk = getattr(run, "pk", None)
        if attach:
            self.attach_grads()
        reducer = self.reducer

        red = _Ready(self, run, reducer) if reducer is not None else None
        run.dw_pending, run.dw_ready_keys, run.dw_count = [], [], 0
        dq = L.zeros(N, H, dtype=F32, device=dev)
        Vout = run.Vout
        Vp = _ru(Vout, 64)
        if gloss is not None and run.labels is not None:
            rows = run.rows_i32
            R = rows.numel()
            if R > 0:
                dlog = torch.empty(R, Vp, dtype=BF16, device=dev)
                gs = gloss.detach().to(F32) if (isinstance(gloss, torch.Tensor) and gloss.is_cuda) else float(gloss)
                ar = torch.arange(R, dtype=torch.int32, device=dev)
                L.ce_bwd_rows(run.logits_c, run.labels_c, ar, Vout, Vp, run.row_lse, run.loss_acc, gs, dlog)
                self._head_bwd(run, rows, dlog, dq)
                del dlog
        if glogits is not None:
            gl = glogits.reshape(B * S, Vout)
            if pk is not None:
                gl = gl.index_select(0, pk.sel)
            dlog = torch.zeros(N, Vp, dtype=BF16, device=dev) if Vp != Vout else torch.empty(N, Vp, dtype=BF16, device=dev)
            dlog[:, :Vout].copy_(gl)
            self._head_bwd(run, torch.arange(N, dtype=torch.int32, device=dev), dlog, dq, all_rows=True)
            del dlog

        def stage_done(key):
            run.dw_ready_keys.append(key)
            self._dw_flush(run, red)

        stage_done("head")
        run.pos_chain = None
        if "deberta.encoder.LayerNorm.weight" in self.G:
            from .attn_bwd import pos_chain_buffers

            run.pos_chain = pos_chain_buffers(self, run, len(run.layers))
        layers = run.layers
        dkv_ops = []
        for _ in range(2):
            sv = layers.pop()
            dq, dkv_op = self._layer_bwd(run, sv, dq)
            dkv_ops.append(dkv_op)
        WkvT = self.Lw[self.nL - 1]["WqkvT"][:, H:]
        dx = dq
        for op in dkv_ops:
            acc = torch.empty(N, H, dtype=F32, device=dev)
            L.gemm(op, WkvT, aux=dx, aux_kind=L.AUX_ADD_F32, out_f32=acc)
            dx = acc
        del dkv_ops
        stage_done(f"layer{self.nL - 1}")
        while layers:
            sv = layers.pop()
            if sv.li == 0 and cfg.conv_kernel_size:
                dx, dcol = self._conv_bwd(run, dx)
                dx, _ = self._layer_bwd(run, sv, dx)
                if pk is None:
                    L.col2im3(dcol, dx, B, S, H, 1)
                else:
                    dcg = torch.zeros(B * S, 3 * H, dtype=F32, device=dev).index_copy_(0, pk.sel, dcol)
                    dxg = torch.zeros(B * S, H, dtype=F32, device=dev)
                    L.col2im3(dcg, dxg, B, S, H, 1)
                    dx.add_(dxg.index_select(0, pk.sel))
                    del dcg, dxg
                stage_done("conv")
            else:
                dx, _ = self._layer_bwd(run, sv, dx)
            stage_done(f"layer{sv.li}")
        self._dw_flush(run, red, force=True)
        if getattr(run, "side_used", False):
            torch.cuda.current_stream().wait_stream(self.side)
        rn = run.rel_norm
        if run.pos_chain is not None:
            from .attn_bwd import pos_table_grads_batched

            dR = pos_table_grads_batched(self, run, run.pos_chain)
            run.pos_chain = None
            L.ln_bwd(dR, rn.t, rn.stats, rn.gamma, dgamma=self.G.get("deberta.encoder.LayerNorm.weight"),
                     dbeta=self.G.get("deberta.encoder.LayerNorm.bias"), ws=self._ln_ws)
        if red:
            red.ready("relln")
        if run.p_hid > 0:
            L.dropout_f32(dx, run.p_hid, run.seed_emb, out_f32=dx)
        en = run.emb_norm
        dt0 = torch.empty(N, H, dtype=F32, device=dev)
        L.ln_bwd(dx, en.t, en.stats, en.gamma, rowmask=en.rowmask, out_dt=dt0,
                 dgamma=self.G.get("deberta.embeddings.LayerNorm.weight"), dbeta=self.G.get("deberta.embeddings.LayerNorm.bias"),
                 ws=self._ln_ws)
        if T:
            if pk is None:
                dv = dt0.view(B, S, H)[:, :T].reshape(B * T, H).contiguous()
            else:
                dv = dt0.index_select(0, (pk.row0[:-1].long()[:, None] + torch.arange(T, device=dev)[None]).reshape(-1))
            Kp = _ru(B * T, 64)
            dvT = torch.empty(H, Kp, dtype=BF16, device=dev)
            vT = torch.empty(self.Fp, Kp, dtype=BF16, device=dev)
            L.transpose_to_bf16(dv, dvT)
            L.transpose_to_bf16(run.video_bf16, vT)
            L.gemm(dvT, vT, aux=self.G["deberta.embeddings.linear_video.weight"], aux_kind=L.AUX_ADD_F32,
                   out_f32=self.G["deberta.embeddings.linear_video.weight"], N=self.F)
            L.colsum(dv, self.G["deberta.embeddings.linear_video.bias"], self._cs_ws)
        if red:
            red.ready("emb")
            red.finish()

    def _conv_bwd(self, run, dout):
        B, S, H, dev = run.B, run.S, self.H, self.dev
        N = run.N
        cn = run.conv_norm
        dt = torch.empty(N, H, dtype=F32, device=dev)
        L.ln_bwd(dout, cn.t, cn.stats, cn.gamma, rowmask=cn.rowmask, out_dt=dt,
                 dgamma=self.G.get("deberta.encoder.conv.LayerNorm.weight"),
                 dbeta=self.G.get("deberta.encoder.conv.LayerNorm.bias"), ws=self._ln_ws)
        dc = torch.empty(N, H, dtype=BF16, device=dev)
        L.dropout_gelu_bwd(dt, run.conv_c, run.p_hid, run.seed_conv, out_bf16=dc)
        dcol = torch.empty(N, 3 * H, dtype=F32, device=dev)
        L.gemm(dc, self.WcT, rowscale=run.mask_f, out_f32=dcol)
        return dt, dcol


class _Ready:

    __slots__ = ("eng", "run", "reducer")

    def __init__(self, eng, run, reducer):
        self.eng, self.run, self.reducer = eng, run, reducer

    def ready(self, key):
        ev = getattr(self.run, "dw_event", None)
        if ev is not None:
            torch.cuda.current_stream().wait_event(ev)
        self.reducer.ready(key)

    def finish(self):
        self.reducer.finish()


@dataclass
class LayerSave:
    li: int = 0
    emd: bool = False
    qkv: torch.Tensor = None
    pqk: torch.Tensor = None
    ctx: torch.Tensor = None
    lse: torch.Tensor = None
    ob: torch.Tensor = None
    z1: torch.Tensor = None
    ln1: NormRef = None
    hpre: torch.Tensor = None
    fb: torch.Tensor = None
    z2: torch.Tensor = None
    ln2: NormRef = None
    seed_pos: int = 0
    seed_att: int = 0
    seed_ad1: int = 0
    seed_ad2: int = 0
    seed_ln1: int = 0
    seed_ln2: int = 0
    psave: torch.Tensor = None
    msave: torch.Tensor = None


@dataclass
class Run:
    B: int
    S: int
    T: int
    Lt: int
    train: bool
    save: bool
    seed_base: int
    p_hid: float
    p_att: float
    p_ad: float
    layers: List[LayerSave] = field(default_factory=list)
    _site: int = 0
    mask: torch.Tensor = None
    labels: torch.Tensor = None
    hidden_out: tuple = None
    seed_word: Optional[torch.Tensor] = None
    want_attn: bool = False
    attn_out: list = field(default_factory=list)
    seed_emb: int = 0
    seed_conv: int = 0
    pk: Optional["Packing"] = None
    N: int = 0

    def __post_init__(self):
        if not self.N:
            self.N = self.B * self.S

    def next_seed(self) -> int:
        self._site += 1
        return (self.seed_base + self._site * 0x85EBCA77) & 0xFFFFFFFFFFFFFFFF


class _StepFn(torch.autograd.Function):

    @staticmethod
    def forward(ctx, engine, run, loss_t, logits_t, *params):
        ctx.engine, ctx.run = engine, run
        ctx.set_materialize_grads(False)
        return loss_t.detach().clone(), logits_t.detach()

    @staticmethod
    def backward(ctx, gloss, glogits):
        eng, run = ctx.engine, ctx.run
        if gloss is None and glogits is None:
            return (None, None, None, None) + tuple(None for _ in eng.order)
        eng.backward(run, gloss, glogits)
        return (None, None, None, None) + tuple(None for _ in eng.order)
```

### frozenbilm_amd/lib.py

```python
from __future__ import annotations

import ctypes as C
import os
from typing import Optional

import torch

HERE = os.path.dirname(os.path.abspath(__file__))
LIB_PATH = os.environ.get("FBL_LIB") or os.path.join(HERE, "libfbl.so")

ACT_NONE, ACT_GELU, ACT_RELU, ACT_GELU_GRAD = 0, 1, 2, 3
AUX_NONE, AUX_ADD_F32, AUX_ADD_BF16, AUX_MUL_DGELU_BF16, AUX_MUL_POS_BF16, AUX_MUL_BF16 = 0, 1, 2, 3, 4, 5
ABI_VERSION = 9

_vp, _i, _l, _f, _u64 = C.c_void_p, C.c_int, C.c_int64, C.c_float, C.c_uint64

SIGNATURES = {
    "fbl_abi_version": (_i, []),
    "fbl_gemm_bf16_nt": (_i, [_vp, _l, _vp, _l, _i, _i, _i, _vp, _vp, _f, _i, _i, _vp, _l, _vp, _vp, _vp, _l, _i, _l, _l,
                              _l, _l, _l, _i, _vp, _l, _vp, _vp]),
    "fbl_adapter_down_fwd": (_i, [_vp, _l, _vp, _l, _i, _i, _i, _vp, _f, _u64, _vp, _vp, _l, _vp]),
    "fbl_dense_adapter_down_fwd": (_i, [_vp, _l, _vp, _l, _i, _i, _i, _i, _vp, _vp, _vp, _l, _f, _u64, _vp, _vp, _l, _vp, _vp]),
    "fbl_adapter_up_resid_fwd": (_i, [_vp, _l, _vp, _l, _i, _i, _i, _vp, _vp, _l, _f, _u64, _vp, _vp, _l, _vp, _vp, _vp, _vp,
                                      _vp, _l, _vp]),
# ... 238 lines not shown
    assert wd.shape[1] == K and z.shape[0] >= M and z.shape[1] >= A
    _chk(load().fbl_adapter_down_fwd(_p(x), ldx, _p(wd), ldw, M, A, K, _p(bias), float(p_drop), int(seed), _seed_dev(), _p(z), ldz,
                                     _stream()), "fbl_adapter_down_fwd")


def dense_adapter_down_fwd(x, wm, bias_m, N1, z, *, y_f32=None, y_bf16=None, p_drop=0.0, seed=0):
    _req(x, torch.bfloat16, "x"); _req(wm, torch.bfloat16, "wm"); _req(z, torch.bfloat16, "z"); _req(bias_m, torch.float32, "bias")
    ldx, ldw, ldz = _rows2d(x, "x"), _rows2d(wm, "wm"), _rows2d(z, "z")
    M, K = x.shape
    A = wm.shape[0] - N1
    assert wm.shape[1] == K and A > 0 and z.shape[0] >= M and z.shape[1] >= A and bias_m.numel() >= N1 + A
    ldy = None
    for o, dt in ((y_f32, torch.float32), (y_bf16, torch.bfloat16)):
        if o is not None:
            _req(o, dt, "y")
            l = _rows2d(o, "y")
            assert ldy is None or ldy == l
            ldy = l
    _chk(load().fbl_dense_adapter_down_fwd(_p(x), ldx, _p(wm), ldw, M, N1, A, K, _p(bias_m), _p(y_f32), _p(y_bf16), ldy or 0,
                                           float(p_drop), int(seed), _seed_dev(), _p(z), ldz, _stream(), _aux_stream()),
         "fbl_dense_adapter_down_fwd")


def adapter_up_resid_fwd(z, wu, bias_u, x, out_t, *, A=None, p_drop=0.0, seed=0, r_plain=None, r_norm=None):
    _req(z, torch.bfloat16, "z"); _req(wu, torch.bfloat16, "wu"); _req(x, torch.bfloat16, "x"); _req(out_t, torch.float32, "out_t")
    ldz, ldw, ldx, ldt = _rows2d(z, "z"), _rows2d(wu, "wu"), _rows2d(x, "x"), _rows2d(out_t, "out_t")
    M, H = x.shape
    A = wu.shape[1] if A is None else A
    assert wu.shape[0] == H and z.shape[0] >= M and z.shape[1] >= A and out_t.shape[0] >= M and out_t.shape[1] >= H
    if bias_u is not None:
        _req(bias_u, torch.float32, "bias_u")
    if (r_plain is None) == (r_norm is None):
        raise ValueError("exactly one of r_plain / r_norm")
    rs = rg = rb = rm = None
    if r_norm is not None:
        rt, rs, rg, rb, rm = r_norm
        for t in (rt, rs, rg, rb):
            _req(t, torch.float32, "r_norm")
        assert rs.is_contiguous() and rs.numel() >= 2 * M
        if rm is not None:
            _req(rm, torch.int32, "rowmask")
    else:
        rt = r_plain
        _req(rt, torch.float32, "r_plain")
    ld_r = _rows2d(rt, "residual")
    assert rt.shape[0] >= M and rt.shape[1] >= H
    _chk(load().fbl_adapter_up_resid_fwd(_p(z), ldz, _p(wu), ldw, M, H, int(A), _p(bias_u), _p(x), ldx, float(p_drop),
                                         int(seed), _seed_dev(), _p(rt), ld_r, _p(rs), _p(rg), _p(rb), _p(rm), _p(out_t), ldt,
                                         _stream()), "fbl_adapter_up_resid_fwd")


def gemm_tn_acc(A, B, out_f32, ws, *, M=None, N=None, K=None, splitk=8):
    _req(A, torch.bfloat16, "A"); _req(B, torch.bfloat16, "B"); _req(out_f32, torch.float32, "out")
    lda, ldb, ldc = _rows2d(A, "A"), _rows2d(B, "B"), _rows2d(out_f32, "out")
    K = min(A.shape[0], B.shape[0]) if K is None else K
    M = A.shape[1] if M is None else M
    N = B.shape[1] if N is None else N
    assert out_f32.shape[0] >= M and out_f32.shape[1] >= N
    _chk(load().fbl_gemm_bf16_tn_acc(_p(A), lda, _p(B), ldb, M, N, K, _p(out_f32), ldc, splitk, _p(ws), ws.numel(),
                                     _stream()), "fbl_gemm_bf16_tn_acc")


ADW_MAX_ADAPTERS, ADW_MAX_SEGMENTS = 16, 24


def adapter_bwd_dw(groups, *, A):
    segs = [sg for g in groups for sg in g[0]]
    assert 0 < len(groups) <= ADW_MAX_ADAPTERS and 0 < len(segs) <= ADW_MAX_SEGMENTS
    N, H = segs[0][0].shape
    Ap = segs[0][1].shape[1]
    strides = []
    for g in groups:
        lds = None
        for dy, z, dz, x in g[0]:
            for t, n in ((dy, "dy"), (z, "z"), (dz, "dz"), (x, "x")):
                _req(t, torch.bfloat16, n)
            assert dy.shape == (N, H) and x.shape == (N, H) and z.shape == (N, Ap) and dz.shape == (N, Ap) and Ap >= A
            l = (_rows2d(dy, "dy"), _rows2d(z, "z"), _rows2d(dz, "dz"), _rows2d(x, "x"))
            assert lds is None or l == lds, "the segments of an adapter share their row strides"
            lds = l
        strides.append(lds)
    for _, dWu, dWd, dbd in groups:
        for o, shp in ((dWu, (H, A)), (dWd, (A, H)), (dbd, (A,))):
            if o is not None:
                _req(o, torch.float32, "out")
                assert tuple(o.shape) == shp and o.is_contiguous(), (tuple(o.shape), shp)
    first = [0]
    for g in groups:
        first.append(first[-1] + len(g[0]))
    seg_first = (C.c_int32 * len(first))(*first)
    tab = lambda ts: (C.c_void_p * len(ts))(*[_p(t) for t in ts])
    ldt = lambda k: (C.c_int64 * len(strides))(*[st[k] for st in strides])
    _chk(load().fbl_adapter_bwd_dw(len(groups), seg_first, tab([s[0] for s in segs]), tab([s[1] for s in segs]),
                                   tab([s[2] for s in segs]), tab([s[3] for s in segs]), ldt(0), ldt(1), ldt(2), ldt(3),
                                   N, H, int(A), Ap, tab([g[1] for g in groups]), tab([g[2] for g in groups]),
                                   tab([g[3] for g in groups]), _stream()), "fbl_adapter_bwd_dw")


def embed_gather(ids, E, vproj, T, out_t):
    B, L = ids.shape
    H = E.shape[1]
    _req(ids, torch.int64, "ids"); _req(E, torch.float32, "E"); _req(out_t, torch.float32, "out_t")
    assert ids.is_contiguous() and E.is_contiguous() and out_t.is_contiguous()
    if vproj is not None:
        _req(vproj, torch.float32, "vproj")
        assert vproj.is_contiguous()
    _chk(load().fbl_embed_gather(_p(ids), _p(E), _p(vproj), B, T, L, H, _p(out_t), _stream()), "fbl_embed_gather")


def ln_fwd(*, y=None, p_drop=0.0, seed=0, r_plain=None, r_norm=None, gamma, beta, eps, rowmask=None, out_t=None,
           out_stats=None, out_bf16=None, out_f32=None, N, H):
    ldy = 0
    if y is not None:
        _req(y, torch.float32, "y")
        ldy = _rows2d(y, "y")
    rt = rs = rg = rb = rm = None
    if r_norm is not None:
        rt, rs, rg, rb, rm = r_norm
    for t in (r_plain, rt, out_t, out_bf16, out_f32):
        if t is not None:
            assert t.is_contiguous()
    _chk(load().fbl_ln_fwd(_p(y), ldy, float(p_drop), int(seed), _seed_dev(), _p(r_plain), _p(rt), _p(rs), _p(rg), _p(rb), _p(rm),
                           _p(gamma), _p(beta), float(eps), _p(rowmask), _p(out_t), _p(out_stats), _p(out_bf16),
                           _p(out_f32), N, H, _stream()), "fbl_ln_fwd")


def ln_materialize(t, stats, gamma, beta, rowmask=None, add_bcast=None, S=1, out_f32=None, out_bf16=None):
    N, H = t.shape
    _chk(load().fbl_ln_materialize(_p(t), _p(stats), _p(gamma), _p(beta), _p(rowmask), _p(add_bcast), S, _p(out_f32),
                                   _p(out_bf16), N, H, _stream()), "fbl_ln_materialize")


def ln_bwd_ws(H, device):
    return torch.empty(load().fbl_ln_bwd_ws_floats(H), dtype=torch.float32, device=device)


def ln_bwd(dout, t, stats, gamma, *, rowmask=None, p_drop=0.0, seed=0, out_dt=None, out_dy_bf16=None, out_dy_f32=None,
           dgamma=None, dbeta=None, dysum=None, ws=None):
    N, H = t.shape
    assert dout.is_contiguous() and t.is_contiguous()
    ld_dyb = _rows2d(out_dy_bf16, "out_dy_bf16") if out_dy_bf16 is not None else 0
    _chk(load().fbl_ln_bwd(_p(dout), _p(rowmask), _p(t), _p(stats), _p(gamma), float(p_drop), int(seed), _seed_dev(), _p(out_dt),
                           _p(out_dy_bf16), _p(out_dy_f32), _p(dgamma), _p(dbeta), _p(dysum), _p(ws), N, H, ld_dyb,
                           _stream()), "fbl_ln_bwd")


def im2col3(x_bf16, out_bf16, B, S, H):
    _chk(load().fbl_im2col3(_p(x_bf16), _p(out_bf16), B, S, H, _stream()), "fbl_im2col3")


def col2im3(dcol, dx, B, S, H, accumulate):
    _chk(load().fbl_col2im3(_p(dcol), _p(dx), B, S, H, int(accumulate), _stream()), "fbl_col2im3")


def dropout_gelu_fwd(c, p_drop, seed, out_f32):
    _chk(load().fbl_dropout_gelu_fwd(_p(c), float(p_drop), int(seed), _seed_dev(), _p(out_f32), c.numel(), _stream()),
         "fbl_dropout_gelu_fwd")


def dropout_gelu_bwd(dy, c, p_drop, seed, out_bf16=None, out_f32=None):
    _chk(load().fbl_dropout_gelu_bwd(_p(dy), _p(c), float(p_drop), int(seed), _seed_dev(), _p(out_bf16), _p(out_f32), c.numel(),
                                     _stream()), "fbl_dropout_gelu_bwd")


def video_stage_f16(feats, row_off, n_rows, T):
    assert feats.dtype == torch.float16 and feats.is_contiguous() and row_off.dtype == torch.int64 and n_rows.dtype == torch.int32
    B, F_ = n_rows.numel(), feats.shape[1]
    video = torch.empty(B, T, F_, dtype=torch.float32, device=feats.device)
    vlen = torch.empty(B, dtype=torch.int64, device=feats.device)
    vmask = torch.empty(B, T, dtype=torch.int64, device=feats.device)
    _chk(load().fbl_video_stage_f16(_p(feats), _p(row_off), _p(n_rows), B, T, F_, _p(video), _p(vlen), _p(vmask), _stream()),
         "fbl_video_stage_f16")
    return video, vlen, vmask


def mask_tokens(ids, labels, special_ids, p, mask_token_id, vocab_size, seed):
    assert ids.dtype == torch.int64 and labels.dtype == torch.int64 and ids.is_contiguous() and labels.is_contiguous()
    assert special_ids.dtype == torch.int64
    _chk(load().fbl_mask_tokens(_p(ids), _p(labels), ids.numel(), _p(special_ids), special_ids.numel(), float(p),
                                int(mask_token_id), int(vocab_size), int(seed), _stream()), "fbl_mask_tokens")


def transpose_batched_bf16(src, src_off, dst, dst_off, rows, cols):
    assert src.dtype == torch.bfloat16 and dst.dtype == torch.bfloat16
    assert src_off.dtype == torch.int64 and dst_off.dtype == torch.int64 and src_off.numel() == dst_off.numel()
    _chk(load().fbl_transpose_batched_bf16(_p(src), _p(src_off), _p(dst), _p(dst_off), src_off.numel(), rows, cols,
                                           _stream()), "fbl_transpose_batched_bf16")


def transpose_to_bf16(x, out, rows=None, cols=None):
    ld = _rows2d(x, "x")
    rows = x.shape[0] if rows is None else rows
    cols = x.shape[1] if cols is None else cols
    assert out.is_contiguous() and out.shape[0] >= cols
    _req(out, torch.bfloat16, "out")
    is_bf = 1 if x.dtype == torch.bfloat16 else 0
    if not is_bf:
        _req(x, torch.float32, "x")
    _chk(load().fbl_transpose_to_bf16(_p(x), is_bf, ld, rows, cols, _p(out), out.shape[1], _stream()),
         "fbl_transpose_to_bf16")


def colsum_ws(cols, device):
    return torch.empty(load().fbl_colsum_ws_floats(cols), dtype=torch.float32, device=device)


def colsum(x, out, ws, rows=None, cols=None):
    ld = _rows2d(x, "x")
    rows = x.shape[0] if rows is None else rows
    cols = x.shape[1] if cols is None else cols
    is_bf = 1 if x.dtype == torch.bfloat16 else 0
    _chk(load().fbl_colsum(_p(x), is_bf, ld, rows, cols, _p(out), _p(ws), _stream()), "fbl_colsum")


def head_strides(B, Sp, nh, head_major):
    if head_major:
        return 64 * B * Sp, Sp, B * Sp
    return 64 * Sp, nh * 64 * Sp, Sp


def head_transpose(v, vt, B, S, Sp, nh, head_major=False):
    ldv = _rows2d(v, "v")
    _req(v, torch.bfloat16, "v"); _req(vt, torch.bfloat16, "vt")
    assert vt.is_contiguous() and vt.numel() == B * nh * 64 * Sp
    sh, sb, sd = head_strides(B, Sp, nh, head_major)
    _chk(load().fbl_head_transpose(_p(v), ldv, _p(vt), B, S, Sp, nh, sh, sb, sd, _stream()), "fbl_head_transpose")


def _row0(row0, B, klen):
    if row0 is None:
        return None
    _req(row0, torch.int32, "row0")
    assert row0.is_contiguous() and row0.numel() == B + 1 and klen is not None
    return _p(row0)


def disent_attn_fwd(q, k, v, pk, pq, relidx, mask, scale, ctx, lse, B, S, Sp, nh, span2, p_drop=0.0, seed=0, klen=None,
                    border=None, lin=0, row0=None, psave=None, msave=None):
    if psave is not None:
        _req(psave, torch.bfloat16, "psave"); _req(msave, torch.float32, "msave")
        assert psave.is_contiguous() and msave.is_contiguous()
        assert psave.numel() == B * nh * Sp * Sp and msave.numel() == B * nh * (Sp // 64) * S
    for t, n in ((q, "q"), (k, "k"), (v, "v"), (pk, "pk"), (pq, "pq"), (ctx, "ctx")):
        _req(t, torch.bfloat16, n)
    _req(relidx, torch.int16, "relidx"); _req(mask, torch.int32, "mask")
    assert relidx.numel() == 2 * S - 1 and mask.is_contiguous()
    ldq, ldk, ldv, ldp, ldo = _rows2d(q, "q"), _rows2d(k, "k"), _rows2d(v, "v"), _rows2d(pk, "pk"), _rows2d(ctx, "ctx")
    assert _rows2d(pq, "pq") == ldp
    _chk(load().fbl_disent_attn_fwd(_p(q), ldq, _p(k), ldk, _p(v), ldv, _p(pk), _p(pq), ldp, _p(relidx),
                                    _p(mask), _p(klen), _p(border), float(scale), float(p_drop), int(seed), _seed_dev(), _p(ctx), ldo,
                                    _p(lse), B, S, Sp, nh, span2, int(lin), _row0(row0, B, klen), _p(psave), _p(msave), _stream()),
         "fbl_disent_attn_fwd")


def disent_attn_probs(q, k, pk, pq, relidx, mask, lse, scale, probs, B, S, nh):
    for t, n in ((q, "q"), (k, "k"), (pk, "pk"), (pq, "pq")):
        _req(t, torch.bfloat16, n)
    _req(relidx, torch.int16, "relidx"); _req(mask, torch.int32, "mask"); _req(lse, torch.float32, "lse"); _req(probs, torch.float32, "probs")
    ldq, ldp = _rows2d(q, "q"), _rows2d(pk, "pk")
    assert _rows2d(k, "k") == ldq and _rows2d(pq, "pq") == ldp and probs.is_contiguous() and probs.numel() == B * nh * S * S
    _chk(load().fbl_disent_attn_probs(_p(q), _p(k), ldq, _p(pk), _p(pq), ldp, _p(relidx), _p(mask), _p(lse), float(scale),
                                      _p(probs), B, S, nh, _stream()), "fbl_disent_attn_probs")


def attn_bwd_prep(q, pq, pk, dO, O, QT, PQT, Dv, B, S, Sp, nh, span2, row0=None, relidx=None, PQX=None, PKX=None):
    ldq, ldp, ldo = _rows2d(q, "q"), _rows2d(pq, "pq"), _rows2d(dO, "dO")
    assert _rows2d(pk, "pk") == ldp and _rows2d(O, "O") == ldo
    for t in (QT, PQT, PQX, PKX):
        if t is not None:
            _req(t, torch.bfloat16, "transposed output")
            assert t.is_contiguous()
    for t in (PQX, PKX):
        if t is not None:
            _req(relidx, torch.int16, "relidx")
            assert t.numel() == nh * 64 * 2 * Sp and relidx.numel() == 2 * S - 1
    _chk(load().fbl_attn_bwd_prep(_p(q), ldq, _p(pq), _p(pk), ldp, _p(dO), _p(O), ldo, _p(QT), _p(PQT), _p(Dv), _p(relidx),
                                  _p(PQX), _p(PKX), B, S, Sp, nh, span2, _row0(row0, B, True), _stream()),
         "fbl_attn_bwd_prep")


def attn_rowdot(dO, O, out, B, S, nh):
    ld = _rows2d(dO, "dO")
    assert _rows2d(O, "O") == ld
    _chk(load().fbl_attn_rowdot(_p(dO), _p(O), ld, _p(out), B, S, nh, _stream()), "fbl_attn_rowdot")


def disent_attn_bwd_ds(q, k, v, dO, pk, pq, relidx, mask, lse, Dv, scale, dV, dS, dST, B, S, Sp, nh, span2,
                       p_drop=0.0, seed=0, klen=None, border=None, lin=0, row0=None):
    ldq = _rows2d(q, "q")
    assert _rows2d(k, "k") == ldq and _rows2d(v, "v") == ldq
    ldo, ldp, lddv = _rows2d(dO, "dO"), _rows2d(pk, "pk"), _rows2d(dV, "dV")
    assert _rows2d(pq, "pq") == ldp
    _chk(load().fbl_disent_attn_bwd_ds(_p(q), _p(k), _p(v), ldq, _p(dO), ldo, _p(pk), _p(pq), ldp,
                                       _p(relidx), _p(mask), _p(klen), _p(border), _p(lse), _p(Dv), float(scale), float(p_drop), int(seed), _seed_dev(),
                                       _p(dV), lddv, _p(dS), _p(dST), B, S, Sp, nh, span2, int(lin), _row0(row0, B, klen), _stream()),
         "fbl_disent_attn_bwd_ds")


def disent_attn_bwd_dspk(psave, msave, q, v, dO, pqx, lse, Dv, scale, dK, dV, dS, dST, B, S, Sp, nh, p_drop=0.0, seed=0, klen=None,
                         border=None, row0=None):
    _req(psave, torch.bfloat16, "psave"); _req(msave, torch.float32, "msave"); _req(pqx, torch.bfloat16, "pqx")
    assert psave.is_contiguous() and msave.is_contiguous() and pqx.is_contiguous()
    assert psave.numel() == B * nh * Sp * Sp and msave.numel() == B * nh * (Sp // 64) * S and pqx.numel() == nh * 64 * 2 * Sp
    ldq, ldv, ldo, lddk, lddv = _rows2d(q, "q"), _rows2d(v, "v"), _rows2d(dO, "dO"), _rows2d(dK, "dK"), _rows2d(dV, "dV")
    _chk(load().fbl_disent_attn_bwd_dspk(_p(psave), _p(msave), _p(q), ldq, _p(v), ldv, _p(dO), ldo, _p(pqx), _p(klen), _p(border),
                                         _p(lse), _p(Dv), float(scale), float(p_drop), int(seed), _seed_dev(), _p(dK), lddk,
                                         _p(dV), lddv, _p(dS), _p(dST), B, S, Sp, nh, _row0(row0, B, klen), _stream()),
         "fbl_disent_attn_bwd_dspk")


def disent_attn_bwd_dq(dS, k, pkx, dQ, B, S, Sp, nh, klen=None, border=None, row0=None):
    _req(dS, torch.bfloat16, "dS"); _req(pkx, torch.bfloat16, "pkx")
    assert dS.is_contiguous() and pkx.is_contiguous() and dS.numel() == B * nh * Sp * Sp and pkx.numel() == nh * 2 * Sp * 64
    ldk, lddq = _rows2d(k, "k"), _rows2d(dQ, "dQ")
    _chk(load().fbl_disent_attn_bwd_dq(_p(dS), _p(k), ldk, _p(pkx), _p(klen), _p(border), _p(dQ), lddq, B, S, Sp, nh,
                                       _row0(row0, B, klen), _stream()), "fbl_disent_attn_bwd_dq")


def attn_pos_grad(neg, Xs, Ys, dlo, dcnt, dcnt_max, out, B, S, Sp, nh, rcnt, klen=None, row0=None):
    E = len(Xs)
    assert E == len(Ys) and E > 0
    ldy = _rows2d(Ys[0], "Y")
    for x, y in zip(Xs, Ys):
        _req(x, torch.bfloat16, "X"); _req(y, torch.bfloat16, "Y")
        assert x.is_contiguous() and x.numel() == B * nh * Sp * Sp and _rows2d(y, "Y") == ldy
    _req(dlo, torch.int16, "dlo"); _req(dcnt, torch.int16, "dcnt"); _req(out, torch.float32, "out")
    assert dlo.numel() == rcnt and dcnt.numel() == rcnt and out.is_contiguous() and out.numel() == E * nh * rcnt * 64
    xp = (C.c_void_p * E)(*[x.data_ptr() for x in Xs])
    yp = (C.c_void_p * E)(*[y.data_ptr() for y in Ys])
    _chk(load().fbl_attn_pos_grad(int(neg), xp, yp, ldy, _p(dlo), _p(dcnt), int(dcnt_max), _p(klen), _row0(row0, B, klen), _p(out),
                                  E, B, S, Sp, nh, int(rcnt), _stream()), "fbl_attn_pos_grad")


def disent_attn_bwd_shear(dST, QT, PQT, relidx, dK, B, S, Sp, nh, span2, klen=None, lin=0, border=None, row0=None):
    lddk = _rows2d(dK, "dK")
    sh, sb, sd = head_strides(B, Sp, nh, True)
    _chk(load().fbl_disent_attn_bwd_shear(_p(dST), _p(QT), sh, sb, sd, _p(PQT), _p(relidx), _p(klen), _p(border), _p(dK), lddk,
                                          int(lin), B, S, Sp, nh, span2, _row0(row0, B, klen), _stream()),
         "fbl_disent_attn_bwd_shear")


def ce_fwd(logits, labels, V, row_lse, loss_sum_cnt):
    ldv = _rows2d(logits, "logits")
    _req(logits, torch.float32, "logits"); _req(labels, torch.int64, "labels")
    _chk(load().fbl_ce_fwd(_p(logits), ldv, _p(labels), logits.shape[0], V, _p(row_lse), _p(loss_sum_cnt), _stream()),
         "fbl_ce_fwd")


def ce_bwd_rows(logits, labels, rows, V, Vp, row_lse, loss_sum_cnt, gscale, dlogits):
    ldv = _rows2d(logits, "logits")
    _req(rows, torch.int32, "rows")
    gdev = None
    if isinstance(gscale, torch.Tensor):
        gdev = gscale.reshape(1)
        _req(gdev, torch.float32, "gscale")
        gscale = 1.0
    _chk(load().fbl_ce_bwd_rows(_p(logits), ldv, _p(labels), _p(rows), rows.numel(), V, Vp, _p(row_lse),
                                _p(loss_sum_cnt), float(gscale), _p(gdev), _p(dlogits), _stream()), "fbl_ce_bwd_rows")


def gather_rows_bf16(x, rows, out):
    ld = _rows2d(x, "x")
    _chk(load().fbl_gather_rows_bf16(_p(x), ld, _p(rows), rows.numel(), x.shape[1], _p(out), _stream()),
         "fbl_gather_rows_bf16")


def scatter_rows_f32(x, rows, out):
    ld = _rows2d(out, "out")
    _chk(load().fbl_scatter_rows_f32(_p(x), _p(rows), rows.numel(), x.shape[1], _p(out), ld, _stream()),
         "fbl_scatter_rows_f32")


_SUMSQ_WS = {}


def sumsq(x, out, ws=None):
    if ws is None:
        ws = _SUMSQ_WS.get(x.device)
        if ws is None:
            ws = _SUMSQ_WS[x.device] = torch.empty(load().fbl_sumsq_ws_floats(), dtype=torch.float32, device=x.device)
    _chk(load().fbl_sumsq(_p(x), x.numel(), _p(out), _p(ws), _stream()), "fbl_sumsq")


def adam_flat(p, g, m, v, lr, beta1, beta2, eps, weight_decay, step, sumsq_t=None, max_norm=0.0, grad_scale=1.0):
    _chk(load().fbl_adam_flat(_p(p), _p(g), _p(m), _p(v), p.numel(), float(lr), float(beta1), float(beta2), float(eps),
                              float(weight_decay), int(step), _p(sumsq_t), float(max_norm), float(grad_scale),
                              _stream()), "fbl_adam_flat")


def cast_bf16(x, out):
    _req(x, torch.float32, "x"); _req(out, torch.bfloat16, "out")
    assert x.is_contiguous() and out.is_contiguous()
    _chk(load().fbl_cast_f32_to_bf16(_p(x), _p(out), x.numel(), _stream()), "fbl_cast_f32_to_bf16")


def dropout_f32(x, p_drop, seed, out_f32=None, out_bf16=None):
    _req(x, torch.float32, "x")
    assert x.is_contiguous()
    _chk(load().fbl_dropout_f32(_p(x), float(p_drop), int(seed), _seed_dev(), _p(out_f32), _p(out_bf16), x.numel(), _stream()),
         "fbl_dropout_f32")


def zero_(t):
    assert t.is_contiguous()
    _chk(load().fbl_zero(_p(t), t.numel() * t.element_size(), _stream()), "fbl_zero")
    return t


def zeros(*shape, dtype, device):
    return zero_(torch.empty(*shape, dtype=dtype, device=device))


def heads_to_rows_bf16(src, dst):
    E, nh, rows, c = src.shape
    assert c == 64 and src.is_contiguous() and dst.shape[0] == E and dst.shape[1] == rows and dst.stride(2) == 1
    assert dst.stride(0) == rows * dst.stride(1)
    _req(src, torch.float32, "src")
    _req(dst, torch.bfloat16, "dst")
    _chk(load().fbl_heads_to_rows_bf16(_p(src), _p(dst), E, nh, rows, dst.stride(1), _stream()), "fbl_heads_to_rows_bf16")


def dropout_sum_f32(x, seeds, p_drop, out, key0=0):
    ns = x.shape[0]
    n = x.numel() // ns
    assert x.is_contiguous() and out.is_contiguous() and out.numel() == n and len(seeds) == ns
    arr = (C.c_uint64 * ns)(*[int(v) & 0xFFFFFFFFFFFFFFFF for v in seeds])
    _chk(load().fbl_dropout_sum_f32(_p(x), n, int(key0), ns, arr, float(p_drop), _seed_dev(), _p(out), _stream()), "fbl_dropout_sum_f32")


def dropout_bf16_(x, p_drop, seed):
    _req(x, torch.bfloat16, "x")
    assert x.is_contiguous()
    _chk(load().fbl_dropout_bf16(_p(x), float(p_drop), int(seed), _seed_dev(), x.numel(), _stream()), "fbl_dropout_bf16")


def mha_fwd(q, k, v, mask, scale, ctx, lse, B, S, nh, p_drop=0.0, seed=0, klen=None, border=None):
    for t, n in ((q, "q"), (k, "k"), (v, "v"), (ctx, "ctx")):
        _req(t, torch.bfloat16, n)
    _req(mask, torch.int32, "mask"); _req(lse, torch.float32, "lse")
    assert mask.is_contiguous() and mask.numel() == B * S and lse.is_contiguous() and lse.numel() == B * nh * S
    for t in (klen, border):
        if t is not None:
            _req(t, torch.int32, "klen/border")
            assert t.is_contiguous() and t.numel() == B
    _chk(load().fbl_mha_fwd(_p(q), _rows2d(q, "q"), _p(k), _rows2d(k, "k"), _p(v), _rows2d(v, "v"), _p(mask), _p(klen), _p(border),
                            float(scale), float(p_drop), int(seed), _seed_dev(), _p(ctx), _rows2d(ctx, "ctx"), _p(lse), B, S, nh,
                            _stream()), "fbl_mha_fwd")


def mha_bwd(q, k, v, dO, mask, lse, Dv, scale, dQ, dK, dV, B, S, nh, p_drop=0.0, seed=0, klen=None, border=None):
    for t, n in ((q, "q"), (k, "k"), (v, "v"), (dO, "dO"), (dQ, "dQ"), (dK, "dK"), (dV, "dV")):
        _req(t, torch.bfloat16, n)
    _req(mask, torch.int32, "mask"); _req(lse, torch.float32, "lse"); _req(Dv, torch.float32, "Dv")
    assert mask.numel() == B * S and lse.numel() == B * nh * S and Dv.numel() == B * nh * S
    _chk(load().fbl_mha_bwd(_p(q), _rows2d(q, "q"), _p(k), _rows2d(k, "k"), _p(v), _rows2d(v, "v"), _p(dO), _rows2d(dO, "dO"),
                            _p(mask), _p(klen), _p(border), _p(lse), _p(Dv), float(scale), float(p_drop), int(seed), _seed_dev(),
                            _p(dQ), _rows2d(dQ, "dQ"), _p(dK), _rows2d(dK, "dK"), _p(dV), _rows2d(dV, "dV"), B, S, nh, _stream()),
         "fbl_mha_bwd")
```

Before: 767.4 samples/s.

## Skip writing transposed dS in saved-P attention backward; read dS by columns for position grads

By default the saved-P attention backward kernel no longer writes the transposed score gradient dS^T, which saves one B×nh×Sp×Sp bf16 store per layer and the memory that holds it. The dPQ position-table gradient kernels get a column-reading mode (neg=2). In that mode they load dS column-wise into a transposed shared-memory image instead of reading rows of dS^T. The trade-off is strided global reads and extra LDS traffic and syncs in the position-gradient kernels, in exchange for less HBM write traffic and smaller LDS use in the dspk kernel.

```diff
diff --git a/frozenbilm_amd/attn_bwd.py b/frozenbilm_amd/attn_bwd.py
--- a/frozenbilm_amd/attn_bwd.py
+++ b/frozenbilm_amd/attn_bwd.py
@@ -75,7 +75,8 @@
         PQX = None
     L.attn_bwd_prep(q, pq, pk, dctx, sv.ctx, QT, PQT, Dv, B, S, Sp, nh, span2, row0=row0, relidx=relidx, PQX=PQX, PKX=PKX)
     dS = torch.empty(B, nh, Sp, Sp, dtype=BF16, device=dev)
-    dST = torch.empty(B, nh, Sp, Sp, dtype=BF16, device=dev)
+    write_dst = (not saved_p) or bool(getattr(eng, "attn_write_dst", True))
+    dST = torch.empty(B, nh, Sp, Sp, dtype=BF16, device=dev) if write_dst else None
     lin = eng.cfg.position_buckets // 2 if eng.cfg.position_buckets > 0 else eng.cfg.att_span - 1
     if saved_p:
         L.disent_attn_bwd_dspk(sv.psave, sv.msave, q, v, dctx, PQX, sv.lse, Dv, scale, dqkv[:, H:2 * H], dqkv[:, 2 * H:], dS, dST,
@@ -102,7 +103,8 @@
     rmin, rcnt, B, Sp = st["rmin"], st["rcnt"], st["B"], st["Sp"]
     dpos = torch.zeros(span2, 2 * H, dtype=F32, device=eng.dev)
     dlo, dcnt, cmax = _delta_ranges(st["S"], eng.cfg, eng.dev, limit=None)
-    for neg, X, Y, col0 in ((0, st["dS"], st["q"], H), (1, st["dST"], st["k"], 0)):
+    dpq = (1, st["dST"]) if st["dST"] is not None else (2, st["dS"])
+    for neg, X, Y, col0 in ((0, st["dS"], st["q"], H), (*dpq, st["k"], 0)):
         d = torch.empty(1, nh, rcnt, 64, dtype=F32, device=eng.dev)
         L.attn_pos_grad(neg, [X], [Y], dlo, dcnt, cmax, d, B, st["S"], Sp, nh, rcnt, klen=st["klen"], row0=st["row0"])
         dpos[rmin:rmin + rcnt, col0:col0 + H].view(rcnt, nh, 64).copy_(d[0].permute(1, 0, 2))
@@ -113,7 +115,7 @@
     rmin, rcnt = _relidx_range(run.S, eng.cfg)
     Sp = (run.S + 63) // 64 * 64
     return dict(X1=[], X2=[], Yq=[], Yk=[], rmin=rmin, rcnt=rcnt, B=run.B, S=run.S, Sp=Sp, n=0, seeds=[], cap=n_exec, klen=None,
-                row0=None)
+                row0=None, neg2=1)
 
 
 def pos_table_grads_batched(eng, run, pc):
@@ -122,7 +124,7 @@
     dev = eng.dev
     dpb = torch.empty(E, rcnt, 2 * H, dtype=BF16, device=dev)
     dlo, dcnt, cmax = _delta_ranges(pc["S"], eng.cfg, dev, limit=None)
-    for neg, kx, ky, col0 in ((0, "X1", "Yq", H), (1, "X2", "Yk", 0)):
+    for neg, kx, ky, col0 in ((0, "X1", "Yq", H), (pc.get("neg2", 1), "X2", "Yk", 0)):
         d = torch.empty(E, nh, rcnt, 64, dtype=F32, device=dev)
         L.attn_pos_grad(neg, pc[kx][:E], pc[ky][:E], dlo, dcnt, cmax, d, B, pc["S"], Sp, nh, rcnt, klen=pc["klen"], row0=pc["row0"])
         L.heads_to_rows_bf16(d, dpb[:, :, col0:col0 + H])
diff --git a/frozenbilm_amd/csrc/attn_bwd.hip b/frozenbilm_amd/csrc/attn_bwd.hip
--- a/frozenbilm_amd/csrc/attn_bwd.hip
+++ b/frozenbilm_amd/csrc/attn_bwd.hip
@@ -462,9 +462,19 @@
   float m, l, D;
 };
 
-template <bool PACKED = false>
+template <bool WT>
+struct PKLds {
+  static constexpr int G2 = WT ? K_G2 : K_STT;
+  static constexpr int TAB = G2 + 64 * LDG2 * 2;
+  static constexpr int ROW = TAB + 16384;
+  static constexpr int TOTAL = ROW + 512;
+};
+static_assert(PKLds<true>::TOTAL == K_TOTAL, "the layout with dS^T is the one above");
+
+template <bool PACKED = false, bool WT = true>
 __global__ __launch_bounds__(256, 2) void attn_bwd_dspk_kernel(BwdPKArgs ka) {
   extern __shared__ __attribute__((aligned(16))) char smem[];
+  constexpr int K_G2 = PKLds<WT>::G2, K_TAB = PKLds<WT>::TAB, K_ROW = PKLds<WT>::ROW;
   const BwdPArgs& a = ka.p;
   const int tid = threadIdx.x, lane = tid & 63;
   const int w = __builtin_amdgcn_readfirstlane(tid >> 6);
@@ -515,7 +525,7 @@
   const __amdgpu_buffer_rsrc_t qr = buf_rsrc(ka.q + rb * ka.ldq + h * 64);
   const __amdgpu_buffer_rsrc_t pr = buf_rsrc(a.psave + sbase + j0);
   const __amdgpu_buffer_rsrc_t dSr = buf_rsrc(a.dS + sbase + j0);
-  const __amdgpu_buffer_rsrc_t dSTr = buf_rsrc(a.dST + sbase + (long)j0 * Sp);
+  const __amdgpu_buffer_rsrc_t dSTr = buf_rsrc(WT ? a.dST + sbase + (long)j0 * Sp : a.dS);
   const uint32_t ldo2 = (uint32_t)(a.ldo * 2), ldq2 = (uint32_t)(ka.ldq * 2);
   const uint32_t po = (uint32_t)((srow * Sp + sch * 8) * 2);
   auto load_tile = [&](int it, PKTileRegs& R) {
@@ -626,7 +636,7 @@
       bf16* gs = g2 + 64 - (w * 16 + c) + g * 4;
 #pragma unroll
       for (int nt = 0; nt < 4; ++nt) {
-        *(bf16x4*)(dstT + (w * 16 + c) * LDV + nt * 16 + g * 4) = dsb[nt];
+        if (WT) *(bf16x4*)(dstT + (w * 16 + c) * LDV + nt * 16 + g * 4) = dsb[nt];
 #pragma unroll
         for (int r = 0; r < 4; ++r) {
           dst[(nt * 16 + g * 4 + r) * LDP + w * 16 + c] = dsb[nt][r];
@@ -656,7 +666,7 @@
     for (int t = 0; t < 2; ++t) {
       const int row = srow + t * 32;
       buf_st16(dSr, po + (uint32_t)(t * 32 * Sp * 2), (uint32_t)(i0 * Sp * 2), *(const bf16x8*)(dst + row * LDP + sch * 8));
-      buf_st16(dSTr, po + (uint32_t)(t * 32 * Sp * 2), (uint32_t)(i0 * 2), *(const bf16x8*)(dstT + row * LDV + sch * 8));
+      if (WT) buf_st16(dSTr, po + (uint32_t)(t * 32 * Sp * 2), (uint32_t)(i0 * 2), *(const bf16x8*)(dstT + row * LDV + sch * 8));
     }
   }
 
@@ -974,9 +984,13 @@
 __host__ __device__ constexpr int pg_pitch(int Sp) { return Sp + 2 * PG_PAD; }
 __host__ __device__ constexpr int pg_buf(int Sp) { return 32 * pg_pitch(Sp) * 2 + 32 * PG_LDY * 2; }
 __host__ __device__ constexpr int pg_smem(int Sp) { return 2 * pg_buf(Sp); }
-
-template <bool NEG, int CM, int NXR, int OCC>
+constexpr int PG_CP = 34;
+__host__ __device__ constexpr int pg_cimg(int Sp) { return (Sp + 2 * PG_PAD) * PG_CP; }
+__host__ __device__ constexpr int pg_cbuf(int Sp) { return pg_cimg(Sp) * 2 + 32 * PG_LDY * 2; }
+
+template <bool NEG, int CM, int NXR, int OCC, bool COL = false>
 __global__ __launch_bounds__(PG_THR, OCC) void pos_grad_kernel(PosGradArgs a) {
+  static_assert(NEG || !COL, "column blocks: dPQ only");
   extern __shared__ __attribute__((aligned(16))) char smem[];
   const int tid = threadIdx.x, lane = tid & 63;
   const int w = __builtin_amdgcn_readfirstlane(tid >> 6);
@@ -987,7 +1001,8 @@
   const int prob = (L8 / nsplit) * 8 + xcd, part = L8 % nsplit;
   if (prob >= a.E * a.nh) return;
   const int e = prob / a.nh, h = prob % a.nh;
-  const int bufsz = pg_buf(Sp);
+  const int bufsz = COL ? pg_cbuf(Sp) : pg_buf(Sp);
+  const int ximg = COL ? pg_cimg(Sp) : 32 * P;
   const bf16* X = a.X[e];
   const bf16* Y = a.Y[e];
   const int ntiles = (a.rcnt + 15) / 16;
@@ -1012,14 +1027,24 @@
 #pragma unroll
     for (int dt = 0; dt < 4; ++dt) acc[u][dt] = (f32x4){0.f, 0.f, 0.f, 0.f};
 
-  for (int id = tid; id < (OCC >= 3 ? 1 : 2) * 32 * 2 * (PG_PAD / 8); id += PG_THR) {
-    const int bsel = id / (32 * 2 * (PG_PAD / 8)), r2 = id % (32 * 2 * (PG_PAD / 8));
-    const int row = r2 / (2 * (PG_PAD / 8)), q = r2 % (2 * (PG_PAD / 8));
-    const int col = q < PG_PAD / 8 ? q * 8 : PG_PAD + Sp + (q - PG_PAD / 8) * 8;
-    *(bf16x8*)((bf16*)(smem + bsel * bufsz) + row * P + col) = (bf16x8){0, 0, 0, 0, 0, 0, 0, 0};
+  if (COL) {
+    constexpr int ZD = PG_PAD * PG_CP / 2;
+    for (int id = tid; id < (OCC >= 3 ? 1 : 2) * 2 * ZD; id += PG_THR) {
+      const int bsel = id / (2 * ZD), r2 = id % (2 * ZD);
+      const int dw = r2 < ZD ? r2 : (PG_PAD + Sp) * (PG_CP / 2) + (r2 - ZD);
+      ((uint32_t*)(smem + bsel * bufsz))[dw] = 0u;
+    }
+  } else {
+    for (int id = tid; id < (OCC >= 3 ? 1 : 2) * 32 * 2 * (PG_PAD / 8); id += PG_THR) {
+      const int bsel = id / (32 * 2 * (PG_PAD / 8)), r2 = id % (32 * 2 * (PG_PAD / 8));
+      const int row = r2 / (2 * (PG_PAD / 8)), q = r2 % (2 * (PG_PAD / 8));
+      const int col = q < PG_PAD / 8 ? q * 8 : PG_PAD + Sp + (q - PG_PAD / 8) * 8;
+      *(bf16x8*)((bf16*)(smem + bsel * bufsz) + row * P + col) = (bf16x8){0, 0, 0, 0, 0, 0, 0, 0};
+    }
   }
   const bf16x8 z8 = (bf16x8){0, 0, 0, 0, 0, 0, 0, 0};
   const int srow = tid >> 3, sch = tid & 7, nq = Sp >> 6;
+  const int c_row = tid >> 2, c_ch = tid & 3;
 
   int b_n = 0, k_n = 0, kl_n = 0;
   auto seek = [&]() {
@@ -1037,10 +1062,16 @@
     const int kl64 = (kl_n + 63) & ~63;
     const long rb = a.row0 ? (long)a.row0[b_n] : (long)b_n * S;
     const int lim = a.row0 ? min(a.row0[b_n + 1] - a.row0[b_n], S) : S;
-    const bf16* Xb = X + (((long)b_n * a.nh + h) * Sp) * Sp + (long)k_n * Sp;
-    const bf16* xr = Xb + (long)srow * Sp + sch * 8;
-#pragma unroll
-    for (int q = 0; q < NXR; ++q) rx[q] = (q < nq && sch * 8 + q * 64 < kl64) ? *(const bf16x8*)(xr + q * 64) : z8;
+    if (COL) {
+      const bf16* xr = X + (((long)b_n * a.nh + h) * Sp) * Sp + (long)c_row * Sp + k_n + c_ch * 8;
+#pragma unroll
+      for (int q = 0; q < NXR; ++q) rx[q] = (q < nq && c_row + q * 64 < kl64) ? *(const bf16x8*)(xr + (long)q * 64 * Sp) : z8;
+    } else {
+      const bf16* Xb = X + (((long)b_n * a.nh + h) * Sp) * Sp + (long)k_n * Sp;
+      const bf16* xr = Xb + (long)srow * Sp + sch * 8;
+#pragma unroll
+      for (int q = 0; q < NXR; ++q) rx[q] = (q < nq && sch * 8 + q * 64 < kl64) ? *(const bf16x8*)(xr + q * 64) : z8;
+    }
     {
       const int pos = k_n + srow;
       ry = (pos < lim) ? *(const bf16x8*)(Y + (rb + pos) * a.ldy + h * 64 + sch * 8) : z8;
@@ -1052,9 +1083,19 @@
   if (have) load_item();
   while (have) {
     bf16* xs = (bf16*)(smem + pb * bufsz);
-    bf16* ys = xs + 32 * P;
+    bf16* ys = xs + ximg;
     if (OCC >= 3) __syncthreads();
-    {
+    if (COL) {
+      uint32_t* xw = (uint32_t*)(xs + (PG_PAD + c_row) * PG_CP + c_ch * 8);
+#pragma unroll
+      for (int q = 0; q < NXR; ++q)
+        if (q < nq) {
+          union { bf16x8 v; uint32_t d[4]; } u4;
+          u4.v = rx[q];
+#pragma unroll
+          for (int i = 0; i < 4; ++i) xw[q * (64 * PG_CP / 2) + i] = u4.d[i];
+        }
+    } else {
       bf16* xw = xs + srow * P + PG_PAD + sch * 8;
 #pragma unroll
       for (int q = 0; q < NXR; ++q)
@@ -1080,18 +1121,21 @@
       const int cmax = NEG ? k0 + 31 + thi[u] : k0 + 31 - tlo[u];
       if (cmax < 0 || cmin >= kl) continue;
       bf16x8 gf;
-      const bf16* xrow = xs + (g * 8) * P + PG_PAD;
+      const bf16* xrow = COL ? xs + PG_PAD * PG_CP + g * 8 : xs + (g * 8) * P + PG_PAD;
       const int cb = NEG ? (k0 + g * 8 + d0[u]) : (k0 + g * 8 - d0[u]);
       if (simple[u]) {
 #pragma unroll
-        for (int q = 0; q < 8; ++q) gf[q] = xrow[q * P + cb + q];
+        for (int q = 0; q < 8; ++q) gf[q] = COL ? xrow[(cb + q) * PG_CP + q] : xrow[q * P + cb + q];
       } else {
         const int lo = -PG_PAD, hi = Sp + PG_PAD - 1;
         bf16 vv[8][CM];
 #pragma unroll
         for (int q = 0; q < 8; ++q)
 #pragma unroll
-          for (int t2 = 0; t2 < CM; ++t2) vv[q][t2] = xrow[q * P + clampi(NEG ? cb + q + t2 : cb + q - t2, lo, hi)];
+          for (int t2 = 0; t2 < CM; ++t2) {
+            const int x = clampi(NEG ? cb + q + t2 : cb + q - t2, lo, hi);
+            vv[q][t2] = COL ? xrow[x * PG_CP + q] : xrow[q * P + x];
+          }
 #pragma unroll
         for (int q = 0; q < 8; ++q) {
           float sum = 0.f;
@@ -1119,9 +1163,11 @@
 constexpr int PGW_PAD = 6;
 __host__ __device__ constexpr int pgw_pitch(int Sp) { return Sp + PGW_PAD; }
 __host__ __device__ constexpr int pgw_smem(int Sp) { return 32 * pgw_pitch(Sp) * 4 + 32 * PG_LDY * 2; }
-
-template <bool NEG>
+__host__ __device__ constexpr int pgw_csmem(int Sp) { return pgw_smem(Sp) + Sp * PG_CP * 2; }
+
+template <bool NEG, bool COL = false>
 __global__ __launch_bounds__(PG_THR, 2) void pos_grad_wide_kernel(PosGradArgs a) {
+  static_assert(NEG || !COL, "column blocks: dPQ only");
   extern __shared__ __attribute__((aligned(16))) char smem[];
   const int tid = threadIdx.x, lane = tid & 63;
   const int w = __builtin_amdgcn_readfirstlane(tid >> 6);
@@ -1134,6 +1180,7 @@
   const int e = prob / a.nh, h = prob % a.nh;
   float* cs = (float*)smem;
   bf16* ys = (bf16*)(smem + 32 * PP * 4);
+  bf16* img = ys + 32 * PG_LDY;
   const bf16* X = a.X[e];
   const bf16* Y = a.Y[e];
   const int ntiles = (a.rcnt + 15) / 16;
@@ -1159,6 +1206,7 @@
   if (tid < 32) cs[tid * PP + 1] = 0.f;
   const bf16x8 z8 = (bf16x8){0, 0, 0, 0, 0, 0, 0, 0};
   const int srow = tid >> 3, sch = tid & 7, nq = Sp >> 6;
+  const int c_row = tid >> 2, c_ch = tid & 3;
 
   int b_n = 0, k_n = 0, kl_n = 0;
   auto seek = [&]() {
@@ -1176,9 +1224,15 @@
     const int kl64 = (kl_n + 63) & ~63;
     const long rb = a.row0 ? (long)a.row0[b_n] : (long)b_n * S;
     const int lim = a.row0 ? min(a.row0[b_n + 1] - a.row0[b_n], S) : S;
-    const bf16* xr = X + (((long)b_n * a.nh + h) * Sp) * Sp + (long)(k_n + srow) * Sp + sch * 8;
-#pragma unroll
-    for (int q = 0; q < 8; ++q) rx[q] = (q < nq && sch * 8 + q * 64 < kl64) ? *(const bf16x8*)(xr + q * 64) : z8;
+    if (COL) {
+      const bf16* xr = X + (((long)b_n * a.nh + h) * Sp) * Sp + (long)c_row * Sp + k_n + c_ch * 8;
+#pragma unroll
+      for (int q = 0; q < 8; ++q) rx[q] = (q < nq && c_row + q * 64 < kl64) ? *(const bf16x8*)(xr + (long)q * 64 * Sp) : z8;
+    } else {
+      const bf16* xr = X + (((long)b_n * a.nh + h) * Sp) * Sp + (long)(k_n + srow) * Sp + sch * 8;
+#pragma unroll
+      for (int q = 0; q < 8; ++q) rx[q] = (q < nq && sch * 8 + q * 64 < kl64) ? *(const bf16x8*)(xr + q * 64) : z8;
+    }
     const int pos = k_n + srow;
     ry = (pos < lim) ? *(const bf16x8*)(Y + (rb + pos) * a.ldy + h * 64 + sch * 8) : z8;
     k_n += 32;
@@ -1187,16 +1241,35 @@
   if (have) load_item();
   while (have) {
     __syncthreads();
+    if (COL) {
+      uint32_t* xw = (uint32_t*)(img + c_row * PG_CP + c_ch * 8);
+#pragma unroll
+      for (int q = 0; q < 8; ++q)
+        if (q < nq) {
+          union { bf16x8 v; uint32_t d[4]; } u4;
+          u4.v = rx[q];
+#pragma unroll
+          for (int i = 0; i < 4; ++i) xw[q * (64 * PG_CP / 2) + i] = u4.d[i];
+        }
+      __syncthreads();
+    }
     {
       float* cw = cs + srow * PP + 2 + sch * 8;
       float carry = 0.f;
 #pragma unroll
       for (int q = 0; q < 8; ++q) {
         if (q < nq) {
+          bf16x8 xv;
+          if (COL) {
+#pragma unroll
+            for (int i = 0; i < 8; ++i) xv[i] = img[(q * 64 + sch * 8 + i) * PG_CP + srow];
+          } else {
+            xv = rx[q];
+          }
           float run[8];
-          run[0] = bf2f(rx[q][0]);
-#pragma unroll
-          for (int i = 1; i < 8; ++i) run[i] = run[i - 1] + bf2f(rx[q][i]);
+          run[0] = bf2f(xv[0]);
+#pragma unroll
+          for (int i = 1; i < 8; ++i) run[i] = run[i - 1] + bf2f(xv[i]);
           float incl = run[7];
 #pragma unroll
           for (int s = 1; s < 8; s <<= 1) {
@@ -1315,7 +1388,7 @@
                                         int B, int S, int Sp, int nh, const int32_t* row0, void* stream) {
   if (S < 1 || S > 512 || Sp < S || Sp % 64) return FBL_ERR_SHAPE;
   if ((ldv % 8) || (ldo % 8) || (ldq % 8) || (lddv % 4) || (lddk % 4)) return FBL_ERR_ALIGN;
-  if (!psave || !msave || !q || !v || !dO || !pqx || !lse || !Dv || !dK || !dV || !dS || !dST) return FBL_ERR_ARG;
+  if (!psave || !msave || !q || !v || !dO || !pqx || !lse || !Dv || !dK || !dV || !dS) return FBL_ERR_ARG;
   if (row0 && !klen) return FBL_ERR_ARG;
   if (B <= 0 || nh <= 0) return 0;
   BwdPKArgs a{{(const bf16*)psave, msave, (const bf16*)v, ldv, (const bf16*)dO, ldo, klen, border, lse, Dv, scale, p_drop, seed,
@@ -1324,13 +1397,21 @@
   attn_debug_init();
   static bool attr_set = false;
   if (!attr_set) {
+    constexpr int K_NOT = PKLds<false>::TOTAL;
     hipError_t e = hipFuncSetAttribute((const void*)attn_bwd_dspk_kernel<false>, hipFuncAttributeMaxDynamicSharedMemorySize, K_TOTAL);
     if (e == hipSuccess) e = hipFuncSetAttribute((const void*)attn_bwd_dspk_kernel<true>, hipFuncAttributeMaxDynamicSharedMemorySize, K_TOTAL);
+    if (e == hipSuccess) e = hipFuncSetAttribute((const void*)attn_bwd_dspk_kernel<false, false>, hipFuncAttributeMaxDynamicSharedMemorySize, K_NOT);
+    if (e == hipSuccess) e = hipFuncSetAttribute((const void*)attn_bwd_dspk_kernel<true, false>, hipFuncAttributeMaxDynamicSharedMemorySize, K_NOT);
     if (e != hipSuccess) return (int)e;
     attr_set = true;
   }
   const dim3 grid((unsigned)(Sp / 64) * nh * B);
-  if (row0)
+  if (!dST) {
+    if (row0)
+      hipLaunchKernelGGL((attn_bwd_dspk_kernel<true, false>), grid, dim3(256), PKLds<false>::TOTAL, (hipStream_t)stream, a);
+    else
+      hipLaunchKernelGGL((attn_bwd_dspk_kernel<false, false>), grid, dim3(256), PKLds<false>::TOTAL, (hipStream_t)stream, a);
+  } else if (row0)
     hipLaunchKernelGGL(attn_bwd_dspk_kernel<true>, grid, dim3(256), K_TOTAL, (hipStream_t)stream, a);
   else
     hipLaunchKernelGGL(attn_bwd_dspk_kernel<false>, grid, dim3(256), K_TOTAL, (hipStream_t)stream, a);
@@ -1400,13 +1481,25 @@
   if (S < 1 || S > 512 || Sp < S || Sp % 64 || rcnt < 1 || rcnt > 1024) return FBL_ERR_SHAPE;
   if (ldy % 8) return FBL_ERR_ALIGN;
   if (!X || !Y || !dlo || !dcnt || !out || dcnt_max < 1) return FBL_ERR_ARG;
+  if (neg != 0 && neg != 1 && neg != 2) return FBL_ERR_ARG;
   if (row0 && !klen) return FBL_ERR_ARG;
   if (E <= 0 || B <= 0 || nh <= 0) return 0;
   for (int e = 0; e < E; ++e)
     if (!X[e] || !Y[e]) return FBL_ERR_ARG;
+  const bool col = neg == 2;
   static const int occ_sw = FBL_ENV_INT("FBL_POSGRAD_OCC", 3);
   const bool occ3 = Sp <= 320 && dcnt_max <= 3 && occ_sw >= 3;
-  const int smem_bytes = occ3 ? pg_buf(Sp) : pg_smem(Sp);
+  const int smem_bytes = col ? (occ3 ? pg_cbuf(Sp) : 2 * pg_cbuf(Sp)) : occ3 ? pg_buf(Sp) : pg_smem(Sp);
+  static int attr_col = 0;
+  if (col && 2 * pg_cbuf(Sp) > attr_col) {
+    const void* fns[3] = {(const void*)pos_grad_kernel<true, 3, 5, 3, true>, (const void*)pos_grad_kernel<true, 3, 8, 2, true>,
+                          (const void*)pos_grad_kernel<true, 8, 8, 2, true>};
+    for (int i = 0; i < 3; ++i) {
+      hipError_t e1 = hipFuncSetAttribute(fns[i], hipFuncAttributeMaxDynamicSharedMemorySize, 2 * pg_cbuf(Sp));
+      if (e1 != hipSuccess) return (int)e1;
+    }
+    attr_col = 2 * pg_cbuf(Sp);
+  }
   static int attr_bytes = 0;
   if (pg_smem(Sp) > attr_bytes) {
     const void* fns[6] = {(const void*)pos_grad_kernel<false, 3, 5, 3>, (const void*)pos_grad_kernel<true, 3, 5, 3>,
@@ -1427,6 +1520,12 @@
     }
     attr_wide = pgw_smem(Sp);
   }
+  static int attr_wide_col = 0;
+  if (wide && col && pgw_csmem(Sp) > attr_wide_col) {
+    hipError_t e1 = hipFuncSetAttribute((const void*)pos_grad_wide_kernel<true, true>, hipFuncAttributeMaxDynamicSharedMemorySize, pgw_csmem(Sp));
+    if (e1 != hipSuccess) return (int)e1;
+    attr_wide_col = pgw_csmem(Sp);
+  }
   const int nsplit = (rcnt + PG_ROWS - 1) / PG_ROWS;
   for (int e0 = 0; e0 < E; e0 += PG_MAX_E) {
     PosGradArgs a{};
@@ -1441,7 +1540,13 @@
     const dim3 grid((unsigned)(((ne * nh + 7) / 8) * 8 * nsplit));
 #define FBL_PG_LAUNCH(NEG_, CM_, NXR_, OCC_) \
   hipLaunchKernelGGL((pos_grad_kernel<NEG_, CM_, NXR_, OCC_>), grid, dim3(PG_THR), smem_bytes, (hipStream_t)stream, a)
-    if (wide) {
+    if (wide && col) {
+      hipLaunchKernelGGL((pos_grad_wide_kernel<true, true>), grid, dim3(PG_THR), pgw_csmem(Sp), (hipStream_t)stream, a);
+    } else if (col) {
+      if (occ3) hipLaunchKernelGGL((pos_grad_kernel<true, 3, 5, 3, true>), grid, dim3(PG_THR), smem_bytes, (hipStream_t)stream, a);
+      else if (dcnt_max <= 3) hipLaunchKernelGGL((pos_grad_kernel<true, 3, 8, 2, true>), grid, dim3(PG_THR), smem_bytes, (hipStream_t)stream, a);
+      else hipLaunchKernelGGL((pos_grad_kernel<true, 8, 8, 2, true>), grid, dim3(PG_THR), smem_bytes, (hipStream_t)stream, a);
+    } else if (wide) {
       if (neg) hipLaunchKernelGGL(pos_grad_wide_kernel<true>, grid, dim3(PG_THR), pgw_smem(Sp), (hipStream_t)stream, a);
       else hipLaunchKernelGGL(pos_grad_wide_kernel<false>, grid, dim3(PG_THR), pgw_smem(Sp), (hipStream_t)stream, a);
     } else if (occ3) {
diff --git a/frozenbilm_amd/engine.py b/frozenbilm_amd/engine.py
--- a/frozenbilm_amd/engine.py
+++ b/frozenbilm_amd/engine.py
@@ -68,7 +68,7 @@
         L.load()
         self.dev = dev
         self.opts = dict(getattr(model, "engine_options", None) or {})
-        unknown = set(self.opts) - {"eager_logits", "side_stream", "fold_dx", "dw_on_side", "fuse_tail", "merge", "dw_group", "attn_save_p"}
+        unknown = set(self.opts) - {"eager_logits", "side_stream", "fold_dx", "dw_on_side", "fuse_tail", "merge", "dw_group", "attn_save_p", "attn_write_dst"}
         if unknown:
             raise ValueError(f"unknown engine_options: {sorted(unknown)}")
         self._build_flat()
@@ -97,6 +97,7 @@
         self.fold_dx = bool(o.get("fold_dx", True))
         self.dw_on_side = bool(o.get("dw_on_side", False))
         self.attn_save_p = bool(o.get("attn_save_p", True))
+        self.attn_write_dst = bool(o.get("attn_write_dst", False))
         self.fuse_tail = bool(o.get("fuse_tail", True))
         L.exclude_from_aux(self.side)
         self.dw_group = max(1, min(L.ADW_MAX_ADAPTERS, int(o.get("dw_group", 16))))
@@ -996,7 +997,10 @@
         if pc is not None:
             pc["seeds"].append(sv.seed_pos)
             pc["n"] += 1
-            pc["X1"].append(st["dS"]); pc["X2"].append(st["dST"]); pc["Yq"].append(st["q"]); pc["Yk"].append(st["k"])
+            x2, neg2 = (st["dST"], 1) if st["dST"] is not None else (st["dS"], 2)
+            assert pc["n"] == 1 or pc["neg2"] == neg2
+            pc["neg2"] = neg2
+            pc["X1"].append(st["dS"]); pc["X2"].append(x2); pc["Yq"].append(st["q"]); pc["Yk"].append(st["k"])
             pc["klen"], pc["row0"] = st["klen"], st["row0"]
         return dqkv
 
diff --git a/frozenbilm_amd/lib.py b/frozenbilm_amd/lib.py
--- a/frozenbilm_amd/lib.py
+++ b/frozenbilm_amd/lib.py
@@ -564,6 +564,11 @@
     _req(psave, torch.bfloat16, "psave"); _req(msave, torch.float32, "msave"); _req(pqx, torch.bfloat16, "pqx")
     assert psave.is_contiguous() and msave.is_contiguous() and pqx.is_contiguous()
     assert psave.numel() == B * nh * Sp * Sp and msave.numel() == B * nh * (Sp // 64) * S and pqx.numel() == nh * 64 * 2 * Sp
+    _req(dS, torch.bfloat16, "dS")
+    assert dS.is_contiguous() and dS.numel() == B * nh * Sp * Sp
+    if dST is not None:
+        _req(dST, torch.bfloat16, "dST")
+        assert dST.is_contiguous() and dST.numel() == B * nh * Sp * Sp
     ldq, ldv, ldo, lddk, lddv = _rows2d(q, "q"), _rows2d(v, "v"), _rows2d(dO, "dO"), _rows2d(dK, "dK"), _rows2d(dV, "dV")
     _chk(load().fbl_disent_attn_bwd_dspk(_p(psave), _p(msave), _p(q), ldq, _p(v), ldv, _p(dO), ldo, _p(pqx), _p(klen), _p(border),
                                          _p(lse), _p(Dv), float(scale), float(p_drop), int(seed), _seed_dev(), _p(dK), lddk,
@@ -580,6 +585,7 @@
 
 
 def attn_pos_grad(neg, Xs, Ys, dlo, dcnt, dcnt_max, out, B, S, Sp, nh, rcnt, klen=None, row0=None):
+    assert int(neg) in (0, 1, 2), neg
     E = len(Xs)
     assert E == len(Ys) and E > 0
     ldy = _rows2d(Ys[0], "Y")
```

Measured after the change: 778.1 samples/s (median of 6 runs). 1.4% higher.
